# lucaspk512/vrdone

Hardware: AMD Instinct MI355X
Metric: subject-object pairs/sec forward (2048 pairs x 256 frames x 512-d) (higher is better)
Workload: dtype f16x3: f32 products as 3 scaled-f16 MFMA products (~22-bit), f32 accumulate; reference-grade: distance to a float64 run of the reference <= 1.4 x the reference's own float32 error (tests/golden/mask_vrd_f64.npz)

## Files before the change

include/vrdone_hip.h:

```cpp
#ifndef VRDONE_HIP_H
#define VRDONE_HIP_H

#include <stdint.h>

#ifdef __cplusplus
extern "C" {
#endif

#define VRD_ABI_VERSION 36

#define VRD_DETERMINISTIC 1
#define VRD_ERR_SCRATCH (-3)
int vrd_scratch_required(int64_t* floats);

enum vrd_act { VRD_ACT_NONE = 0, VRD_ACT_RELU = 1, VRD_ACT_GELU = 2 };

enum vrd_pair_format { VRD_PAIR_NONE = 0, VRD_PAIR_BF16 = 1, VRD_PAIR_F16 = 2 };
#define VRD_F16_ACT_EXP 4

enum vrd_kernel_id {
    VRD_K_GEMM = 0, VRD_K_LAYERNORM = 1, VRD_K_DWCONV_LN = 2, VRD_K_LOCAL_ATTN = 3,
    VRD_K_ATTN_SMALL = 4, VRD_K_ATTN_FLASH = 5, VRD_K_POOL = 6, VRD_K_MASK_HEAD = 7,
    VRD_K_TRANSPOSE = 8, VRD_K_POSTPROC = 9, VRD_K_GEMM_X3 = 10, VRD_K_GEMM_X3_DMA = 11, VRD_K_GEMM_X3_BIG = 12,
    VRD_K_BACKWARD = 13,
// ... 15 lines not shown
                   float* dst, int64_t ld_dst, int out_pair , int T_src, const int32_t* src_batch,
                   void* stream);
typedef struct {
    const float* const* src;
    const int32_t* lens;
    int32_t P, C_in, T, V, Cc, S, E;
    float* vis;
    float* clip;
    float* so_box;
    float* ent;
    int32_t pair_wide;
} vrd_pack_args;
int vrd_pack_pairs(const vrd_pack_args* a, void* stream);

typedef struct {
    const float* vis;
    const float* clip;
    const float* boxes;
    const int64_t* s_row;
    const int64_t* o_row;
    const int32_t* lens;
    int32_t P, T, V, Cc, stride;
    float w, h;
    float* out_vis;
    float* out_clip;
    float* out_so_box;
    float* out_ent;
    int32_t pair_wide;
    const float* seq_wh;
} vrd_gather_args;
int vrd_gather_pairs(const vrd_gather_args* a, void* stream);

typedef struct {
    const float* vis;
    const float* clip;
    const float* boxes;
    const int64_t* s_row;
    const int64_t* o_row;
    const int32_t* lens;
    const int32_t* lead;
    const float* seq_wh;
    const int32_t* seg_lo;
    const int32_t* seg_hi;
    int32_t P, G, T, V, Cc, stride;
    float* out_vis;
    float* out_clip;
    float* out_so_box;
    float* out_ent;
    uint8_t* out_mask;
    float* out_targets;
    int32_t pair_wide;
} vrd_gather_train_args;
int vrd_gather_train(const vrd_gather_train_args* a, void* stream);

typedef struct {
    const float* streams;
    const float* snippets;
    const int64_t* stream_row;
    const int32_t* lens;
    int32_t P, T, D, L, piece, reach;
    float* out;
} vrd_assemble_args;
int vrd_assemble_pairs(const vrd_assemble_args* a, void* stream);

int vrd_btc_to_bct(const float* src, int64_t ld_src, int B, int C, int T, float* dst, void* stream);

typedef struct {
    const float* A;  int64_t lda;
    const float* W;
    const float* bias;
    float* C;  int64_t ldc;
    int64_t M;  int32_t N;  int32_t Cin;  int32_t taps;  int32_t T;
    int32_t act;
    const uint8_t* row_mask;
    const float* scale;
    const float* res;  int64_t ldres;  int32_t res_masked;
    const float* res2;  int64_t ldres2;
    const uint16_t* W_split;
    int32_t a_pair_width;
    int32_t c_pair;
    const int32_t* row_blocks;
    const int32_t* row_blocks_active;
    int32_t row_block_seg_len;
    int32_t split_fmt;
    const float* w_scale;
    const float* a_scale;
    int32_t products;
} vrd_gemm_args;
int vrd_gemm(const vrd_gemm_args* a, void* stream);
int vrd_gemm_family(const vrd_gemm_args* a);
int vrd_gemm_batch(const vrd_gemm_args* a, int count, void* stream);

int vrd_row_blocks(const uint8_t* mask, int64_t rows, int seg_len, int32_t* order, int32_t* n_active, void* stream);

typedef struct {
    const float* x;
    int64_t ldx;
    int64_t rows;
    int Cin, taps, T, N;
    const float* w;
    const float* bias;
    const uint8_t* row_mask;
    const float* gamma;
    const float* beta;
    int relu;
    float* y;
    int64_t ldy;
    int out_pair;
} vrd_conv_ln_args;
int vrd_conv_ln(const vrd_conv_ln_args* a, void* stream);

int vrd_layernorm(const float* x, int64_t ldx, float* y, int64_t ldy, int64_t rows, int C,
                  const float* gamma, const float* beta, int relu,
                  const float* post_add, int64_t ld_add, int add_period, int out_pair , void* stream);

#define VRD_MAX_SEGS 32
typedef struct {
    int32_t count;
    int32_t n[VRD_MAX_SEGS];
    int32_t T[VRD_MAX_SEGS];
    int64_t row[VRD_MAX_SEGS];
} vrd_row_segs;

typedef struct {
    const float* x;  int64_t ldx;
    const float* x_up;  int64_t ldx_up;
    int32_t B, Tin, C, ksize, stride, group_in;
    const uint8_t* mask_out;
    int32_t n_out;
    const float* w[3];
    const float* bias[3];
    const float* gamma[3];
    const float* beta[3];
    int32_t relu[3];
    float* y[3];
    int64_t ldy[3];
    int32_t out_pair[3];
    const float* pre_gamma;
    const float* pre_beta;
    const float* packed[3];
    const vrd_row_segs* segs;
} vrd_dwconv_ln_args;
int vrd_dwconv_ln(const vrd_dwconv_ln_args* a, void* stream);

int vrd_local_attn(const float* q, const float* k, const float* v, int64_t ld,
                   const uint8_t* mask, const float* rel_pe, int B, int T, int C, int n_head, int half_win,
                   float* out, int64_t ldo, int out_pair, void* stream);
int vrd_local_attn_segs(const float* q, const float* k, const float* v, int64_t ld,
                        const uint8_t* mask, const float* rel_pe, const vrd_row_segs* segs, int C, int n_head, int half_win,
                        float* out, int64_t ldo, int out_pair, void* stream);

int vrd_attention(const float* q, int64_t ldq, const float* k, const float* v, int64_t ldkv,
                  const uint8_t* kv_mask, int B, int Tq, int Tk, int n_head, int head_dim,
                  float* out, int64_t ldo, int algo, int out_pair, void* stream);

int vrd_attention_pair(const float* q, int64_t ldq, const float* k, const float* v, int64_t ldkv,
                       const uint8_t* kv_mask, const uint8_t* q_mask, int B, int Tq, int Tk, int n_head, int head_dim,
                       float* out, int64_t ldo, int out_pair, int pair_fmt, void* stream, int products);

int vrd_maxpool_mask(const float* x, int64_t ldx, int B, int Tin, int C, const uint8_t* mask_in,
                     float* y, int64_t ldy, uint8_t* mask_out, void* stream);

int vrd_mask_head(const float* emb, int64_t ld_emb, const float* feat, int64_t ld_feat,
                  const uint8_t* out_mask, int B, int Q, int T, int Dp, float fill,
                  float* seg, void* stream);

int vrd_postprocess(const float* logits, const float* masks, const int32_t* valid_len,
                    int P, int Q, int K1, int T, int topk,
                    float* top_score, int32_t* top_cat, int32_t* seg_first, int32_t* seg_last,
                    void* stream);

typedef struct {
    const float* cand;
    const float* s_score;
    const float* o_score;
    const int32_t* so_offset;
    const int32_t* so_start;
    const int32_t* so_end;
    const int32_t* video_pairs;
    int32_t n_videos, max_video_pairs, Q, k, feat_stride, pred_min_frames, n_max_pair;
    int32_t* out_count;
    int32_t* out_index;
    float* out_score;
} vrd_select_args;
int vrd_select_triplets(const vrd_select_args* a, void* stream);


int vrd_gemm_wgrad(const float* G, int64_t ldg, const float* X, int64_t ldx, const uint8_t* row_mask, int64_t M, int N, int Cin,
                   int taps, int T, float* dW, float* scratch, int64_t scratch_floats, void* stream, int flags);

int vrd_gemm_wgrad_x3(const float* G, int64_t ldg, const float* X, int64_t ldx, const uint8_t* row_mask, int64_t M, int N, int Cin,
                      int taps, int T, float* dW, float* dbias, float* scratch, int64_t scratch_floats, const float* g_scale,
                      void* stream, int flags);

#define VRD_ABSMAX_SCALE_FLOATS 516
int vrd_absmax_scale(const float* x, int64_t ldx, int64_t rows, int cols, float* scale, void* stream);

int vrd_colsum(const float* a, int64_t lda, const float* b, int64_t ldb, int b_cstride, int b_coffset, int b_rstride, int shift,
               int T, const uint8_t* row_mask, const float* row_scale, int64_t rows, int C, float* out, float* scratch,
               int64_t scratch_floats, void* stream, int flags);

int vrd_dwconv_wgrad(const float* dD, int64_t lddd, const float* x, int64_t ldx, int ksize, int stride, int group_in, int T,
                     const uint8_t* row_mask, int64_t rows, int C, float* dw, float* dbias, float* scratch, int64_t scratch_floats,
                     void* stream, int flags);

int vrd_rowcol_scale(const float* v, int64_t ldv, int64_t rows, int C, const float* col_scale, const float* row_scale,
                     const uint8_t* row_mask, const float* res, int64_t ldres, int res_masked, const float* res2, int64_t ldres2,
                     float* out, int64_t ldo, void* stream);

int vrd_activation(const float* x, int64_t ldx, const float* dy, int64_t lddy, int64_t rows, int C, int act, float* out, int64_t ldo,
            void* stream);

int vrd_layernorm_bwd(const float* x, int64_t ldx, const float* dy, int64_t lddy, int64_t rows, int C, const float* gamma,
                      const float* beta, int relu, float* dx, int64_t lddx, float* dgamma, float* dbeta, float* scratch,
                      int64_t scratch_floats, void* stream, int flags);

typedef struct {
    const float* dD[3];  int64_t lddd[3];
    const float* w[3];
    int32_t n_out, B, Tin, C, ksize, stride, group_in;
    const uint8_t* mask_out;
    float* dx;  int64_t lddx;
    float* dx_up;  int64_t lddx_up;
} vrd_dwconv_bwd_args;
// ... 89 lines not shown
```

vrdone_amd/_hip.py:

```python
import ctypes as C
import os

_HERE = os.path.dirname(os.path.abspath(__file__))
LIB_PATH = os.environ.get("VRDONE_HIP_LIB") or os.path.join(_HERE, "csrc", "libvrdone_hip.so")

ACT_NONE, ACT_RELU, ACT_GELU = 0, 1, 2
PAIR_NONE, PAIR_BF16, PAIR_F16 = 0, 1, 2
F16_ACT_EXP = 4
ABSMAX_SCALE_FLOATS = 516
ADAMW_GROUP_FLOATS = 8
(K_GEMM, K_LAYERNORM, K_DWCONV_LN, K_LOCAL_ATTN, K_ATTN_SMALL, K_ATTN_FLASH, K_POOL, K_MASK_HEAD,
 K_TRANSPOSE, K_POSTPROC, K_GEMM_X3, K_GEMM_X3_DMA, K_GEMM_X3_BIG, K_BACKWARD, K_COUNT) = range(15)
KERNEL_NAMES = ["gemm_f32_mfma", "layernorm", "dwconv_ln", "local_attn", "attn_small", "attn_flash",
                "maxpool_mask", "mask_head", "transpose", "postprocess", "gemm_x3_mfma", "gemm_x3_dma",
                "gemm_x3_big", "backward"]
assert len(KERNEL_NAMES) == K_COUNT

c_f32p = C.c_void_p
c_u8p = C.c_void_p
c_i32p = C.c_void_p


class CriterionArgs(C.Structure):
    _fields_ = [("logits", C.c_void_p * 4), ("masks", C.c_void_p * 4),
                ("n_layers", C.c_int32), ("B", C.c_int32), ("Q", C.c_int32), ("K1", C.c_int32), ("T", C.c_int32), ("G", C.c_int32),
                ("out_valid", C.c_void_p), ("tgt_ids", C.c_void_p), ("tgt_masks", C.c_void_p), ("owner", C.c_void_p),
                ("segs", C.c_void_p), ("scale_range", C.c_float), ("alpha", C.c_float), ("gamma", C.c_float),
                ("w_class", C.c_float), ("w_mask", C.c_float), ("w_dice", C.c_float)]


class CriterionGrads(C.Structure):
    _fields_ = [("logits", C.c_void_p * 4), ("masks", C.c_void_p * 4)]


class GemmArgs(C.Structure):
    _fields_ = [("A", c_f32p), ("lda", C.c_int64), ("W", c_f32p), ("bias", c_f32p),
                ("C", c_f32p), ("ldc", C.c_int64),
                ("M", C.c_int64), ("N", C.c_int32), ("Cin", C.c_int32), ("taps", C.c_int32), ("T", C.c_int32),
                ("act", C.c_int32), ("row_mask", c_u8p), ("scale", c_f32p),
                ("res", c_f32p), ("ldres", C.c_int64), ("res_masked", C.c_int32),
                ("res2", c_f32p), ("ldres2", C.c_int64), ("W_split", C.c_void_p),
                ("a_pair_width", C.c_int32), ("c_pair", C.c_int32),
                ("row_blocks", C.c_void_p), ("row_blocks_active", C.c_void_p), ("row_block_seg_len", C.c_int32),
                ("split_fmt", C.c_int32), ("w_scale", c_f32p), ("a_scale", c_f32p), ("products", C.c_int32)]


MAX_SEGS = 32


class RowSegs(C.Structure):
    _fields_ = [("count", C.c_int32), ("n", C.c_int32 * MAX_SEGS), ("T", C.c_int32 * MAX_SEGS), ("row", C.c_int64 * MAX_SEGS)]

    _made = {}

    @classmethod
    def of(cls, segs):
        key = tuple(segs)
        s = cls._made.get(key)
        if s is None:
            assert 1 <= len(segs) <= MAX_SEGS
            if len(cls._made) > 4096:
                cls._made.clear()
            s = cls._made[key] = cls()
            s.count = len(segs)
            for i, (row, n, T) in enumerate(segs):
                s.row[i], s.n[i], s.T[i] = row, n, T
        return s


class DwconvLnArgs(C.Structure):
    _fields_ = [("x", c_f32p), ("ldx", C.c_int64), ("x_up", c_f32p), ("ldx_up", C.c_int64),
                ("B", C.c_int32), ("Tin", C.c_int32), ("C", C.c_int32), ("ksize", C.c_int32),
                ("stride", C.c_int32), ("group_in", C.c_int32),
                ("mask_out", c_u8p), ("n_out", C.c_int32),
                ("w", c_f32p * 3), ("bias", c_f32p * 3), ("gamma", c_f32p * 3), ("beta", c_f32p * 3),
                ("relu", C.c_int32 * 3), ("y", c_f32p * 3), ("ldy", C.c_int64 * 3), ("out_pair", C.c_int32 * 3),
                ("pre_gamma", c_f32p), ("pre_beta", c_f32p), ("packed", c_f32p * 3), ("segs", C.POINTER(RowSegs))]


class ConvLnArgs(C.Structure):
    _fields_ = [("x", c_f32p), ("ldx", C.c_int64), ("rows", C.c_int64),
                ("Cin", C.c_int32), ("taps", C.c_int32), ("T", C.c_int32), ("N", C.c_int32),
                ("w", c_f32p), ("bias", c_f32p), ("row_mask", c_u8p), ("gamma", c_f32p), ("beta", c_f32p),
                ("relu", C.c_int32), ("y", c_f32p), ("ldy", C.c_int64), ("out_pair", C.c_int32)]


class PackArgs(C.Structure):
    _fields_ = [("src", C.c_void_p), ("lens", C.c_void_p),
                ("P", C.c_int32), ("C_in", C.c_int32), ("T", C.c_int32), ("V", C.c_int32), ("Cc", C.c_int32),
                ("S", C.c_int32), ("E", C.c_int32),
                ("vis", c_f32p), ("clip", c_f32p), ("so_box", c_f32p), ("ent", c_f32p), ("pair_wide", C.c_int32)]


class DwconvBwdArgs(C.Structure):
    _fields_ = [("dD", c_f32p * 3), ("lddd", C.c_int64 * 3), ("w", c_f32p * 3),
                ("n_out", C.c_int32), ("B", C.c_int32), ("Tin", C.c_int32), ("C", C.c_int32), ("ksize", C.c_int32),
                ("stride", C.c_int32), ("group_in", C.c_int32),
                ("mask_out", c_u8p), ("dx", c_f32p), ("lddx", C.c_int64), ("dx_up", c_f32p), ("lddx_up", C.c_int64)]


class BmmArgs(C.Structure):
    _fields_ = [("A", c_f32p), ("a_z0", C.c_int64), ("a_z1", C.c_int64), ("a_row", C.c_int64), ("a_col", C.c_int64),
                ("B", c_f32p), ("b_z0", C.c_int64), ("b_z1", C.c_int64), ("b_row", C.c_int64), ("b_col", C.c_int64),
                ("C", c_f32p), ("c_z0", C.c_int64), ("c_z1", C.c_int64), ("c_row", C.c_int64), ("c_col", C.c_int64),
                ("Z0", C.c_int32), ("Z1", C.c_int32), ("M", C.c_int32), ("N", C.c_int32), ("K", C.c_int32),
                ("alpha", C.c_float), ("accumulate", C.c_int32)]


class SplitJob(C.Structure):
    _fields_ = [("src", c_f32p), ("out", C.c_void_p), ("R", C.c_int32), ("Q", C.c_int32), ("taps", C.c_int32), ("fmt", C.c_int32),
                ("sr", C.c_int64), ("st", C.c_int64), ("sq", C.c_int64), ("scale", c_f32p)]


class GatherArgs(C.Structure):
    _fields_ = [("vis", c_f32p), ("clip", c_f32p), ("boxes", c_f32p), ("s_row", C.c_void_p), ("o_row", C.c_void_p),
                ("lens", C.c_void_p), ("P", C.c_int32), ("T", C.c_int32), ("V", C.c_int32), ("Cc", C.c_int32),
                ("stride", C.c_int32), ("w", C.c_float), ("h", C.c_float),
                ("out_vis", c_f32p), ("out_clip", c_f32p), ("out_so_box", c_f32p), ("out_ent", c_f32p),
                ("pair_wide", C.c_int32), ("seq_wh", c_f32p)]


class GatherTrainArgs(C.Structure):
    _fields_ = [("vis", c_f32p), ("clip", c_f32p), ("boxes", c_f32p), ("s_row", C.c_void_p), ("o_row", C.c_void_p),
                ("lens", C.c_void_p), ("lead", C.c_void_p), ("seq_wh", c_f32p), ("seg_lo", C.c_void_p), ("seg_hi", C.c_void_p),
                ("P", C.c_int32), ("G", C.c_int32), ("T", C.c_int32), ("V", C.c_int32), ("Cc", C.c_int32), ("stride", C.c_int32),
                ("out_vis", c_f32p), ("out_clip", c_f32p), ("out_so_box", c_f32p), ("out_ent", c_f32p), ("out_mask", c_u8p),
                ("out_targets", c_f32p), ("pair_wide", C.c_int32)]


class SelectArgs(C.Structure):
    _fields_ = [("cand", c_f32p), ("s_score", c_f32p), ("o_score", c_f32p), ("so_offset", c_i32p), ("so_start", c_i32p),
                ("so_end", c_i32p), ("video_pairs", c_i32p),
                ("n_videos", C.c_int32), ("max_video_pairs", C.c_int32), ("Q", C.c_int32), ("k", C.c_int32),
                ("feat_stride", C.c_int32), ("pred_min_frames", C.c_int32), ("n_max_pair", C.c_int32),
                ("out_count", c_i32p), ("out_index", c_i32p), ("out_score", c_f32p)]


class AssembleArgs(C.Structure):
    _fields_ = [("streams", c_f32p), ("snippets", c_f32p), ("stream_row", C.c_void_p), ("lens", C.c_void_p),
                ("P", C.c_int32), ("T", C.c_int32), ("D", C.c_int32), ("L", C.c_int32), ("piece", C.c_int32), ("reach", C.c_int32),
                ("out", c_f32p)]


_SIGNATURES = {
    "vrd_abi_version": (C.c_int, []),
    "vrd_last_error": (C.c_char_p, []),
    "vrd_f16_range_flag": (C.c_int, [C.POINTER(C.c_void_p)]),
    "vrd_prof_enable": (C.c_int, [C.c_int]),
    "vrd_prof_reset": (C.c_int, []),
    "vrd_prof_read": (C.c_int, [C.c_int, C.POINTER(C.c_double), C.POINTER(C.c_int64), C.POINTER(C.c_double),
                                C.POINTER(C.c_double)]),
    "vrd_prof_read_skipped": (C.c_int, [C.c_int, C.POINTER(C.c_double)]),
    "vrd_prof_select": (C.c_int, [C.c_uint64]),
    "vrd_bct_to_btc": (C.c_int, [c_f32p, C.c_int, C.c_int, C.c_int, C.c_int, C.c_int, c_f32p, C.c_int64, C.c_int, C.c_int, c_i32p,
                                 C.c_void_p]),
    "vrd_btc_to_bct": (C.c_int, [c_f32p, C.c_int64, C.c_int, C.c_int, C.c_int, c_f32p, C.c_void_p]),
    "vrd_pack_pairs": (C.c_int, [C.POINTER(PackArgs), C.c_void_p]),
    "vrd_gather_pairs": (C.c_int, [C.POINTER(GatherArgs), C.c_void_p]),
    "vrd_gather_train": (C.c_int, [C.POINTER(GatherTrainArgs), C.c_void_p]),
    "vrd_assemble_pairs": (C.c_int, [C.POINTER(AssembleArgs), C.c_void_p]),
# ... 146 lines not shown
```

vrdone_amd/csrc/vrd_gemm.hip:

```cpp
#include "vrd_common.h"
#include "vrd_gemm_epilogue.h"

namespace {

using vrd::f32x16;

constexpr int BM = 128, BN = 128;
constexpr int LDM = 132;

constexpr size_t lds_bytes(int bk) { return (size_t)4 * bk * LDM * sizeof(float); }

template <bool VEC, int TAPS>
__device__ __forceinline__ void load_a(const vrd_gemm_args& p, int64_t r, int t_in_seq, int k, int K, float (&v)[4]) {
    v[0] = v[1] = v[2] = v[3] = 0.f;
    if (r >= p.M) return;
    if (VEC) {
        if (k >= K) return;
        int tap = 0, ci = k;
        if (TAPS == 3) {
            tap = (k >= p.Cin) + (k >= 2 * p.Cin);
            ci = k - tap * p.Cin;
            int tt = t_in_seq + tap - 1;
            if (tt < 0 || tt >= p.T) return;
        }
// ... 154 lines not shown
    constexpr size_t lds = lds_bytes(BK);
    if (lds > 48 * 1024)
        if (int rc = vrd::reserve_lds(reinterpret_cast<const void*>(kern), lds, "vrd_gemm")) return rc;
    hipLaunchKernelGGL(kern, dim3(tiles_m * tiles_n), dim3(256), lds, s, a, tiles_m, tiles_n, a.c_pair == VRD_PAIR_F16 ? vrd::range_flag() : nullptr);
    return 0;
}

template <int BK, bool STAGED>
int launch_bk(const vrd_gemm_args& a, bool vec, int tiles_m, int tiles_n, hipStream_t s) {
    if (a.taps == 1) return vec ? launch_variant<true, 1, BK, STAGED>(a, tiles_m, tiles_n, s)
                                : launch_variant<false, 1, BK, STAGED>(a, tiles_m, tiles_n, s);
    return vec ? launch_variant<true, 3, BK, STAGED>(a, tiles_m, tiles_n, s)
               : launch_variant<false, 3, BK, STAGED>(a, tiles_m, tiles_n, s);
}

}

namespace vrd {
double take_f32_skipped_flops() {
    unsigned long long v = 0, zero = 0;
    if (hipMemcpyFromSymbol(&v, HIP_SYMBOL(g_f32_skipped_kn), sizeof(v)) != hipSuccess) return 0.0;
    (void)hipMemcpyToSymbol(HIP_SYMBOL(g_f32_skipped_kn), &zero, sizeof(zero));
    return 2.0 * BM * (double)v;
}
int launch_gemm_x3(const vrd_gemm_args& a, bool staged, hipStream_t s);
bool gemm_x3_dma_ok(const vrd_gemm_args& a, bool staged);
int launch_gemm_x3_dma(const vrd_gemm_args& a, hipStream_t s);
int launch_gemm_x3_big(const vrd_gemm_args& a, hipStream_t s);
int launch_gemm_x3_big_batch(const vrd_gemm_args* a, int count, hipStream_t s);
}

namespace {
struct X3Choice {
    bool x3, dma, big;
};
X3Choice choose_x3(const vrd_gemm_args* a, bool vec, bool staged) {
    const int K = a->Cin * a->taps;
    const bool x3 = a->a_pair_width > 0 || (a->W_split && vec && (K % 32 == 0) && aligned16(a->W_split));
    static const int dma_env = [] { const char* e = getenv("VRD_X3_DMA"); return e ? atoi(e) : 1; }();
    static const int64_t dma_min_tiles = [] { const char* e = getenv("VRD_X3_DMA_MIN_TILES"); return e ? atoll(e) : 512; }();
    const bool dma = x3 && dma_env && vrd::gemm_x3_dma_ok(*a, staged) &&
                     ((a->M + 127) / 128) * ((a->N + 255) / 256) >= dma_min_tiles;
    static const int64_t big_min_tiles = [] { const char* e = getenv("VRD_X3_BIG_MIN_TILES"); return e ? atoll(e) : 512; }();
    const bool big = dma && a->N >= 256 && K >= 96 && vrd::gemm_epilogue_lean_ok(*a) &&
                     (a->taps == 1 || a->T >= 32) &&
                     (a->products != 1 || (a->Cin % 64 == 0 && K >= 192)) &&
                     (reinterpret_cast<uintptr_t>(a->A) & 127u) == 0 && (reinterpret_cast<uintptr_t>(a->W_split) & 127u) == 0 &&
                     ((a->M + 255) / 256) * ((a->N + 255) / 256) >= big_min_tiles;
    return X3Choice{x3, dma, big};
}
}

namespace {
int validate_gemm_args(const vrd_gemm_args* a) {
    VRD_CHECK_ARG(a->A && a->W && a->C, "vrd_gemm: null operand");
    VRD_CHECK_ARG(a->M >= 0 && a->N > 0 && a->Cin > 0, "vrd_gemm: bad sizes M=%lld N=%d Cin=%d",
                  (long long)a->M, a->N, a->Cin);
    VRD_CHECK_ARG(a->taps == 1 || a->taps == 3, "vrd_gemm: taps must be 1 or 3 (got %d)", a->taps);
    VRD_CHECK_ARG(a->taps == 1 || (a->T > 0 && a->M % a->T == 0),
                  "vrd_gemm: k=3 conv needs M (%lld) to be a multiple of T (%d)", (long long)a->M, a->T);
    VRD_CHECK_ARG(a->lda >= a->Cin && a->ldc >= a->N, "vrd_gemm: leading dimension too small");
    VRD_CHECK_ARG(a->act >= 0 && a->act <= 2, "vrd_gemm: bad activation %d", a->act);
    VRD_CHECK_ARG(!a->res || a->ldres >= a->N, "vrd_gemm: ldres too small");
    VRD_CHECK_ARG(!a->res2 || a->ldres2 >= a->N, "vrd_gemm: ldres2 too small");
    VRD_CHECK_ARG(!a->c_pair || (a->N % 32 == 0 && a->ldc % 32 == 0 && aligned16(a->C)),
                  "vrd_gemm: pair output needs N %% 32 == 0 and rows that start on a 128-byte block");
    VRD_CHECK_ARG(a->a_pair_width == 0 || (a->W_split && a->Cin % 32 == 0 && a->lda % 32 == 0 &&
                                           aligned16(a->A) && aligned16(a->W_split)),
                  "vrd_gemm: pair-row A needs W_split, Cin %% 32 == 0 and rows that start on a 128-byte block");
    VRD_CHECK_ARG(a->split_fmt == 0 || a->split_fmt == VRD_PAIR_BF16 || a->split_fmt == VRD_PAIR_F16, "vrd_gemm: bad split_fmt %d", a->split_fmt);
    VRD_CHECK_ARG(a->split_fmt != VRD_PAIR_F16 || !a->W_split || a->w_scale, "vrd_gemm: a VRD_PAIR_F16 W_split needs w_scale");
    VRD_CHECK_ARG(a->c_pair == VRD_PAIR_NONE || a->c_pair == VRD_PAIR_BF16 || a->c_pair == VRD_PAIR_F16, "vrd_gemm: bad c_pair %d", a->c_pair);
    VRD_CHECK_ARG(!a->a_scale || (a->split_fmt == VRD_PAIR_F16 && a->a_pair_width == 0),
                  "vrd_gemm: a_scale goes with f32-row A in the VRD_PAIR_F16 format");
    VRD_CHECK_ARG(!a->c_pair || !a->W_split || a->c_pair == (a->split_fmt ? a->split_fmt : (int)VRD_PAIR_BF16),
                  "vrd_gemm: pair output (format %d) of a split-precision GEMM must be in its operand format (%d)", a->c_pair, a->split_fmt);
    VRD_CHECK_ARG(a->products == 0 || a->products == 1 || a->products == 3, "vrd_gemm: products must be 0, 1 or 3 (got %d)", a->products);
    VRD_CHECK_ARG(a->products != 1 || (a->split_fmt == VRD_PAIR_F16 && a->W_split),
                  "vrd_gemm: the one-product form (products = 1) needs a VRD_PAIR_F16 W_split (split_fmt %d)", a->split_fmt);
    VRD_CHECK_ARG(!a->row_blocks || (a->row_blocks_active && a->M % 32 == 0 && a->row_block_seg_len >= 8 &&
                                     a->row_block_seg_len % 8 == 0),
                  "vrd_gemm: a row-block list needs its active counts, M %% 32 == 0 and a segment length that is a multiple of 8 (M = %lld, seg_len %d)",
                  (long long)a->M, a->row_block_seg_len);
    return 0;
}
}

static bool gemm_vec(const vrd_gemm_args* a) { return (a->Cin % 4 == 0) && (a->lda % 4 == 0) && aligned16(a->A) && aligned16(a->W); }
static bool gemm_staged(const vrd_gemm_args* a) {
    return (a->ldc % 4 == 0) && aligned16(a->C) && (!a->res || (a->ldres % 4 == 0 && aligned16(a->res))) &&
           (!a->res2 || (a->ldres2 % 4 == 0 && aligned16(a->res2)));
}

extern "C" int vrd_gemm_family(const vrd_gemm_args* a) {
    VRD_CHECK_ARG(a != nullptr, "vrd_gemm_family: null args");
    if (validate_gemm_args(a)) return -1;
    const X3Choice pick = choose_x3(a, gemm_vec(a), gemm_staged(a));
    return pick.big ? VRD_K_GEMM_X3_BIG : pick.dma ? VRD_K_GEMM_X3_DMA : (pick.x3 ? VRD_K_GEMM_X3 : VRD_K_GEMM);
}

extern "C" int vrd_gemm(const vrd_gemm_args* a, void* stream) {
    VRD_CHECK_ARG(a != nullptr, "vrd_gemm: null args");
    if (int rc = validate_gemm_args(a)) return rc;
    if (a->M == 0) return 0;
    const int64_t tiles_m64 = (a->M + BM - 1) / BM;
    const int tiles_n = (a->N + BN - 1) / BN;
    VRD_CHECK_ARG(tiles_m64 * tiles_n < (int64_t)1 << 31, "vrd_gemm: grid too large");
    const int tiles_m = (int)tiles_m64;
    const int K = a->Cin * a->taps;
    const bool vec = gemm_vec(a), staged = gemm_staged(a);
    static const int bk_env = [] { const char* e = getenv("VRD_GEMM_BK"); return e ? atoi(e) : 0; }();
    const int bk = bk_env == 32 ? 32 : 16;
    hipStream_t s = static_cast<hipStream_t>(stream);
    const double flops = 2.0 * (double)a->M * a->N * K;
    const double bytes = 4.0 * ((double)a->M * a->Cin + (double)a->N * K + (double)a->M * a->N *
                                (1.0 + (a->res ? 1.0 : 0.0) + (a->res2 ? 1.0 : 0.0)));
    const X3Choice pick = choose_x3(a, vec, staged);
    const bool x3 = pick.x3, dma = pick.dma, big = pick.big;
    vrd::ProfScope prof(big ? VRD_K_GEMM_X3_BIG : dma ? VRD_K_GEMM_X3_DMA : (x3 ? VRD_K_GEMM_X3 : VRD_K_GEMM), s, flops, bytes);
    if (x3) {
        int rc3 = big ? vrd::launch_gemm_x3_big(*a, s)
                      : dma ? vrd::launch_gemm_x3_dma(*a, s) : vrd::launch_gemm_x3(*a, staged, s);
        if (rc3) return rc3;
        VRD_LAUNCH_CHECK();
        return 0;
    }
    vrd_gemm_args f = *a;
    f.split_fmt = 0;
    f.products = 0;
    f.w_scale = nullptr;
    f.a_scale = nullptr;
    VRD_CHECK_ARG(!f.c_pair || f.c_pair == VRD_PAIR_BF16 || f.c_pair == VRD_PAIR_F16, "vrd_gemm: bad c_pair");
    int rc;
    if (bk == 32) rc = staged ? launch_bk<32, true>(f, vec, tiles_m, tiles_n, s) : launch_bk<32, false>(f, vec, tiles_m, tiles_n, s);
    else          rc = staged ? launch_bk<16, true>(f, vec, tiles_m, tiles_n, s) : launch_bk<16, false>(f, vec, tiles_m, tiles_n, s);
    if (rc) return rc;
    VRD_LAUNCH_CHECK();
    return 0;
}

extern "C" int vrd_gemm_batch(const vrd_gemm_args* a, int count, void* stream) {
    VRD_CHECK_ARG(a != nullptr && count >= 1 && count <= 4, "vrd_gemm_batch: 1..4 problems (got %d)", count);
    for (int i = 0; i < count; ++i)
        if (int rc = validate_gemm_args(&a[i])) return rc;
    for (int i = 1; i < count; ++i)
        VRD_CHECK_ARG((a[i].products == 1) == (a[0].products == 1), "vrd_gemm_batch: every problem needs the same products (%d vs %d)",
                      a[i].products, a[0].products);
    bool same = count > 1 && a[0].M > 0;
    for (int i = 1; i < count && same; ++i) {
        const vrd_gemm_args &x = a[i], &y = a[0];
        same = x.lda == y.lda && x.ldc == y.ldc && x.M == y.M && x.N == y.N && x.Cin == y.Cin && x.taps == y.taps && x.T == y.T &&
               x.act == y.act && x.row_mask == y.row_mask && x.scale == y.scale && x.res == y.res && x.ldres == y.ldres &&
               x.res_masked == y.res_masked && x.res2 == y.res2 && x.ldres2 == y.ldres2 && x.a_pair_width == y.a_pair_width &&
               x.c_pair == y.c_pair && x.row_blocks == y.row_blocks && x.row_blocks_active == y.row_blocks_active &&
               x.row_block_seg_len == y.row_block_seg_len && (x.bias != nullptr) == (y.bias != nullptr) &&
               (x.W_split != nullptr) == (y.W_split != nullptr) && x.split_fmt == y.split_fmt;
    }
    static const int batch_env = [] { const char* e = getenv("VRD_GEMM_BATCH"); return e ? atoi(e) : 1; }();
    if (same && batch_env) {
        bool all_big = true;
        for (int i = 0; i < count && all_big; ++i) {
            const vrd_gemm_args* p = &a[i];
            if (!(p->A && p->W && p->C && p->lda >= p->Cin && p->ldc >= p->N)) { all_big = false; break; }
            const bool vec = (p->Cin % 4 == 0) && (p->lda % 4 == 0) && aligned16(p->A) && aligned16(p->W);
            const bool staged = (p->ldc % 4 == 0) && aligned16(p->C) && (!p->res || (p->ldres % 4 == 0 && aligned16(p->res))) &&
                                (!p->res2 || (p->ldres2 % 4 == 0 && aligned16(p->res2)));
            all_big = choose_x3(p, vec, staged).big && (!p->c_pair || (p->N % 32 == 0 && p->ldc % 32 == 0)) &&
                      (!p->row_blocks || (p->row_blocks_active && p->row_block_seg_len >= 8 && p->row_block_seg_len % 8 == 0));
        }
        if (all_big) {
            hipStream_t s = static_cast<hipStream_t>(stream);
            const int K = a[0].Cin * a[0].taps;
            const double flops = 2.0 * (double)a[0].M * a[0].N * K * count;
            const double bytes = 4.0 * count * ((double)a[0].M * a[0].Cin + (double)a[0].N * K + (double)a[0].M * a[0].N *
                                                (1.0 + (a[0].res ? 1.0 : 0.0) + (a[0].res2 ? 1.0 : 0.0)));
            vrd::ProfScope prof(VRD_K_GEMM_X3_BIG, s, flops, bytes);
            int rc = vrd::launch_gemm_x3_big_batch(a, count, s);
            if (rc) return rc;
            VRD_LAUNCH_CHECK();
            return 0;
        }
    }
    for (int i = 0; i < count; ++i) {
        int rc = vrd_gemm(&a[i], stream);
        if (rc) return rc;
    }
    return 0;
}
```

vrdone_amd/csrc/vrd_gemm_epilogue.h:

```cpp
#pragma once
#include "vrd_common.h"
#include <type_traits>

namespace vrd {

using f32x16 = __attribute__((ext_vector_type(16))) float;
constexpr int STG_PITCH = 64;

typedef float f32x4_t __attribute__((ext_vector_type(4)));
struct acc32q {
    f32x4_t b[2][2];
};
__device__ __forceinline__ void acc_clear(f32x16& a) {
#pragma unroll
    for (int e = 0; e < 16; ++e) a[e] = 0.f;
}
__device__ __forceinline__ void acc_clear(acc32q& a) {
#pragma unroll
    for (int i = 0; i < 2; ++i)
#pragma unroll
        for (int j = 0; j < 2; ++j)
#pragma unroll
            for (int e = 0; e < 4; ++e) a.b[i][j][e] = 0.f;
}
template <typename Fn>
__device__ __forceinline__ void forall32(const f32x16& a, int lane, Fn&& f) {
    const int li = lane & 31, lh = lane >> 5;
#pragma unroll
    for (int e = 0; e < 16; ++e) f((e & 3) + 8 * (e >> 2) + 4 * lh, li, a[e]);
}
template <typename Fn>
__device__ __forceinline__ void forall32(const acc32q& a, int lane, Fn&& f) {
    const int lc = lane & 15, lq = lane >> 4;
#pragma unroll
    for (int bi = 0; bi < 2; ++bi)
#pragma unroll
        for (int bj = 0; bj < 2; ++bj)
#pragma unroll
            for (int j = 0; j < 4; ++j) f(16 * bi + 4 * lq + j, 16 * bj + lc, a.b[bi][bj][j]);
}

__device__ __forceinline__ float epilogue_value(const vrd_gemm_args& p, float v, float mk, float scale, float r1, float rmk,
                                                float r2) {
    if (p.act == VRD_ACT_RELU) v = fmaxf(v, 0.f);
    else if (p.act == VRD_ACT_GELU) v = gelu_erf(v);
    return v * mk * scale + r1 * rmk + r2;
}

struct EpiCols {
    float bias[4], scale[4];
    float alpha;
};
__device__ __forceinline__ float acc_alpha(const vrd_gemm_args& p) {
    if (!(p.split_fmt == VRD_PAIR_F16 && p.w_scale)) return 1.0f;
    const float alpha = uniform_load(p.w_scale);
    return (p.a_scale && p.a_pair_width == 0) ? alpha * F16_ACT_SCALE * uniform_load(p.a_scale + 1) : alpha;
}
__device__ __forceinline__ EpiCols load_epi_cols(const vrd_gemm_args& p, int nw, int lane) {
    EpiCols c;
    c.alpha = acc_alpha(p);
    const int n = nw + (lane & 15) * 4;
#pragma unroll
    for (int j = 0; j < 4; ++j) c.bias[j] = 0.f, c.scale[j] = 1.f;
    if (n + 3 < p.N) {
        if (p.bias) {
            const float4 b = gload4(p.bias + n);
            c.bias[0] = b.x, c.bias[1] = b.y, c.bias[2] = b.z, c.bias[3] = b.w;
        }
        if (p.scale) {
            const float4 b = gload4(p.scale + n);
            c.scale[0] = b.x, c.scale[1] = b.y, c.scale[2] = b.z, c.scale[3] = b.w;
        }
    }
    return c;
}

__device__ __forceinline__ EpiCols load_epi_cols_async(const vrd_gemm_args& p, int nw, int lane) {
    EpiCols c;
    c.alpha = acc_alpha(p);
    const int n = nw + (lane & 15) * 4;
    float4 b = make_float4(0.f, 0.f, 0.f, 0.f), sc = make_float4(1.f, 1.f, 1.f, 1.f);
    if (n + 3 < p.N) {
        if (p.bias) asm volatile("global_load_dwordx4 %0, %1, off" : "=v"(b) : "v"(p.bias + n) : "memory");
        if (p.scale) asm volatile("global_load_dwordx4 %0, %1, off" : "=v"(sc) : "v"(p.scale + n) : "memory");
    }
    c.bias[0] = b.x, c.bias[1] = b.y, c.bias[2] = b.z, c.bias[3] = b.w;
    c.scale[0] = sc.x, c.scale[1] = sc.y, c.scale[2] = sc.z, c.scale[3] = sc.w;
    return c;
}

template <bool ROWIN, int ACT, int SLAB, int ROWS, typename Transposer>
__device__ __forceinline__ void gemm_epilogue_lean_tr(const vrd_gemm_args& p, Transposer&& transpose_into, float* stg, int64_t mw,
                                                      int64_t mw1, int nw, int lane, const EpiCols& cols, unsigned* rflag = nullptr) {
    RangeTrack rt;
    const int64_t hop = mw1 - (mw + 32);
    const int c4 = (lane & 15) * 4, rb0 = lane >> 4;
    const int n = nw + c4;
    const int64_t m_lane = mw + rb0;
    const bool pair = p.c_pair != 0;
    char* const c_lane = reinterpret_cast<char*>(p.C + m_lane * p.ldc) + (pair ? pair_index(n) * 2 : n * 4);
    const float* const r1_lane = (ROWIN && p.res) ? p.res + m_lane * p.ldres + n : nullptr;
    const float* const r2_lane = (ROWIN && p.res2) ? p.res2 + m_lane * p.ldres2 + n : nullptr;
    const unsigned char* const mk_lane = (ROWIN && p.row_mask) ? p.row_mask + m_lane : nullptr;
    const int64_t c_step = p.ldc * 16, r1_step = p.ldres * 4, r2_step = p.ldres2 * 4;
    const int64_t c_hop = hop * p.ldc * 4;
    struct RowIn {
        unsigned char mb[4];
        float4 r1[4], r2[4];
    };
    auto fetch = [&](int pass) {
        RowIn in;
        if (ROWIN) {
            if (p.row_mask) {
#pragma unroll
                for (int j = 0; j < 4; ++j) in.mb[j] = *as_global(mk_lane + pass * 16 + 4 * j + (pass >= 2 ? hop : 0));
            }
            if (p.res) {
#pragma unroll
                for (int j = 0; j < 4; ++j)
                    in.r1[j] = gload4(r1_lane + (pass * 4 + j) * r1_step + (pass >= 2 ? hop * p.ldres : 0));
            }
            if (p.res2) {
#pragma unroll
                for (int j = 0; j < 4; ++j)
                    in.r2[j] = gload4(r2_lane + (pass * 4 + j) * r2_step + (pass >= 2 ? hop * p.ldres2 : 0));
            }
        }
        return in;
    };
    constexpr int NPASS = ROWS / 16;
    RowIn q0 = fetch(0), q1 = fetch(1);
    unsigned rd_addr[4];
    {
        typedef __attribute__((address_space(3))) const float* lds_cf;
#pragma unroll
        for (int j = 0; j < 4; ++j) rd_addr[j] = (unsigned)reinterpret_cast<uintptr_t>((lds_cf)(stg + (rb0 + 4 * j) * STG_PITCH + (c4 ^ (16 * j))));
    }
    transpose_into(stg, SLAB == 64 ? -1 : 0);
#pragma unroll
    for (int pass = 0; pass < NPASS; ++pass) {
        if (SLAB == 32 && pass == 2) transpose_into(stg, 1);
        const RowIn cur = q0;
        q0 = q1;
        if (pass + 2 < NPASS) q1 = fetch(pass + 2);
        float v[4][4];
        float4 tr[4];
        {
            constexpr int PASS_OFF = (SLAB == 64 ? 1 : 0);
            const int poff = (PASS_OFF ? pass : (pass & 1)) * 16 * STG_PITCH * 4;
            asm volatile("ds_read_b128 %0, %4 offset:%8\n\tds_read_b128 %1, %5 offset:%8\n\tds_read_b128 %2, %6 offset:%8\n\tds_read_b128 %3, %7 offset:%8\n\t"
                         "s_waitcnt lgkmcnt(0)"
                         : "=&v"(tr[0]), "=&v"(tr[1]), "=&v"(tr[2]), "=&v"(tr[3])
                         : "v"(rd_addr[0]), "v"(rd_addr[1]), "v"(rd_addr[2]), "v"(rd_addr[3]), "n"(poff)
                         : "memory");
        }
#pragma unroll
        for (int j = 0; j < 4; ++j) {
            const float4 t = tr[j];
            v[j][0] = fmaf(t.x, cols.alpha, cols.bias[0]), v[j][1] = fmaf(t.y, cols.alpha, cols.bias[1]);
            v[j][2] = fmaf(t.z, cols.alpha, cols.bias[2]), v[j][3] = fmaf(t.w, cols.alpha, cols.bias[3]);
        }
        if (ACT == VRD_ACT_GELU) {
#pragma unroll
            for (int j = 0; j < 4; ++j)
#pragma unroll
                for (int c = 0; c < 4; c += 2) {
                    f32x2_t t2;
                    t2.x = v[j][c], t2.y = v[j][c + 1];
                    t2 = gelu_erf2(t2);
                    v[j][c] = t2.x, v[j][c + 1] = t2.y;
                }
        }
        if (ROWIN) {
            float mk[4] = {1.f, 1.f, 1.f, 1.f};
            if (p.row_mask) {
#pragma unroll
                for (int j = 0; j < 4; ++j) mk[j] = (float)cur.mb[j];
            }
            if (p.row_mask || p.scale) {
#pragma unroll
                for (int j = 0; j < 4; ++j)
#pragma unroll
                    for (int c = 0; c < 4; ++c) v[j][c] *= mk[j] * cols.scale[c];
            }
            if (p.res) {
#pragma unroll
                for (int j = 0; j < 4; ++j) {
                    const float rmk = p.res_masked ? mk[j] : 1.f;
                    v[j][0] += cur.r1[j].x * rmk, v[j][1] += cur.r1[j].y * rmk;
                    v[j][2] += cur.r1[j].z * rmk, v[j][3] += cur.r1[j].w * rmk;
                }
            }
            if (p.res2) {
#pragma unroll
                for (int j = 0; j < 4; ++j) {
                    v[j][0] += cur.r2[j].x, v[j][1] += cur.r2[j].y;
                    v[j][2] += cur.r2[j].z, v[j][3] += cur.r2[j].w;
                }
            }
        }
        if (pair) {
            if (p.c_pair == VRD_PAIR_F16) {
#pragma unroll
                for (int j = 0; j < 4; ++j) {
                    char* const rowp = c_lane + (pass * 4 + j) * c_step + (pass >= 2 ? c_hop : 0);
                    f16x4_t h, l;
                    split_n<true>(v[j], h, l, &rt);
                    *as_global(reinterpret_cast<f16x4_t*>(rowp)) = h;
                    *as_global(reinterpret_cast<f16x4_t*>(rowp + 64)) = l;
                }
            } else {
#pragma unroll
                for (int j = 0; j < 4; ++j) {
                    char* const rowp = c_lane + (pass * 4 + j) * c_step + (pass >= 2 ? c_hop : 0);
                    bf16x4_t h, l;
                    split_n<false>(v[j], h, l);
                    *as_global(reinterpret_cast<bf16x4_t*>(rowp)) = h;
                    *as_global(reinterpret_cast<bf16x4_t*>(rowp + 64)) = l;
                }
            }
        } else {
#pragma unroll
            for (int j = 0; j < 4; ++j)
                gstore4(c_lane + (pass * 4 + j) * c_step + (pass >= 2 ? c_hop : 0), make_float4(v[j][0], v[j][1], v[j][2], v[j][3]));
        }
    }
    if (p.c_pair == VRD_PAIR_F16) rt.report(rflag, RANGE_GEMM_OUT);
}

template <bool ROWIN, int ACT, int SLAB = 64>
__device__ __forceinline__ void gemm_epilogue_lean16(const vrd_gemm_args& p, const f32x4_t (&acc)[4][4], float* stg, int64_t mw,
                                                     int64_t mw1, int nw, int lane, const EpiCols& cols, unsigned* rflag = nullptr) {
    const int lc = lane & 15, lq = lane >> 4;
    gemm_epilogue_lean_tr<ROWIN, ACT, SLAB, 64>(
        p,
        [&](float* slab, int half) {
#pragma unroll
            for (int ti = 0; ti < 4; ++ti) {
                if (half >= 0 && (ti >> 1) != half) continue;
                const int r0 = half < 0 ? ti * 16 : (ti & 1) * 16;
#pragma unroll
                for (int tj = 0; tj < 4; ++tj)
#pragma unroll
                    for (int j = 0; j < 4; ++j) slab[(r0 + 4 * lq + j) * STG_PITCH + (tj ^ lq) * 16 + lc] = acc[ti][tj][j];
            }
        },
        stg, mw, mw1, nw, lane, cols, rflag);
}

inline bool gemm_epilogue_lean_ok(const vrd_gemm_args& a) {
    auto al16 = [](const void* q) { return (reinterpret_cast<uintptr_t>(q) & 15u) == 0; };
    return a.M % 64 == 0 && a.N % 64 == 0 && (a.act == VRD_ACT_NONE || a.act == VRD_ACT_GELU) &&
           !(a.act == VRD_ACT_GELU && (a.row_mask || a.scale || a.res || a.res2)) && al16(a.bias) && al16(a.scale);
}

template <bool STAGED, int SLAB_ROWS = 32, typename Acc>
__device__ __forceinline__ void gemm_epilogue(const vrd_gemm_args& p, const Acc (&acc)[2][2], float* smem, int64_t mw,
                                              int nw, int wave, int lane, unsigned* rflag = nullptr, int64_t mw1 = -1) {
    if (mw1 < 0) mw1 = mw + 32;
    auto rowbase = [&](int mi) { return mi ? mw1 : mw; };
    RangeTrack rt;
    constexpr bool SWZ = std::is_same<Acc, acc32q>::value;
    if (STAGED) {
        float* stg = smem + wave * (SLAB_ROWS * STG_PITCH);
        const int c4 = (lane & 15) * 4, rb0 = lane >> 4;
        const int n = nw + c4;
        const bool nfull = n + 3 < p.N;
        const float alpha = acc_alpha(p);
        float bias[4] = {0.f, 0.f, 0.f, 0.f}, scale[4] = {1.f, 1.f, 1.f, 1.f};
        if (nfull && ((reinterpret_cast<uintptr_t>(p.bias) | reinterpret_cast<uintptr_t>(p.scale)) & 15) == 0) {
            if (p.bias) {
                const float4 b = *reinterpret_cast<const float4*>(p.bias + n);
                bias[0] = b.x, bias[1] = b.y, bias[2] = b.z, bias[3] = b.w;
            }
            if (p.scale) {
                const float4 b = *reinterpret_cast<const float4*>(p.scale + n);
                scale[0] = b.x, scale[1] = b.y, scale[2] = b.z, scale[3] = b.w;
            }
        } else {
#pragma unroll
            for (int j = 0; j < 4; ++j)
                if (n + j < p.N) {
                    if (p.bias) bias[j] = p.bias[n + j];
                    if (p.scale) scale[j] = p.scale[n + j];
                }
        }
        const bool row_inputs = p.row_mask || p.res || p.res2;
        const bool ragged = __any(n < p.N && !nfull);
        struct RowIn {
            float mk[4];
            float4 r1[4], r2[4];
        };
        auto fetch = [&](int pass) {
            RowIn in;
#pragma unroll
            for (int j = 0; j < 4; ++j) {
                in.mk[j] = 1.f;
                in.r1[j] = make_float4(0.f, 0.f, 0.f, 0.f);
                in.r2[j] = in.r1[j];
            }
            if (!row_inputs) return in;
            const int64_t mr = rowbase(pass >> 1) + rb0 + (pass & 1) * 16;
            if (!ragged) {
                const int nc = n < p.N ? n : 0;
                unsigned char mb[4];
                int64_t mc[4];
#pragma unroll
                for (int j = 0; j < 4; ++j) mc[j] = (mr + 4 * j < p.M) ? mr + 4 * j : p.M - 1;
                if (p.row_mask) {
#pragma unroll
                    for (int j = 0; j < 4; ++j) mb[j] = p.row_mask[mc[j]];
                }
                if (p.res) {
#pragma unroll
                    for (int j = 0; j < 4; ++j) in.r1[j] = *reinterpret_cast<const float4*>(p.res + mc[j] * p.ldres + nc);
                }
                if (p.res2) {
#pragma unroll
                    for (int j = 0; j < 4; ++j) in.r2[j] = *reinterpret_cast<const float4*>(p.res2 + mc[j] * p.ldres2 + nc);
                }
                if (p.row_mask) {
#pragma unroll
                    for (int j = 0; j < 4; ++j) in.mk[j] = (float)mb[j];
                }
                return in;
            }
#pragma unroll
            for (int j = 0; j < 4; ++j) {
                const int64_t m = mr + 4 * j;
                const bool ok = m < p.M && n < p.N;
// ... 126 lines not shown
```

vrdone_amd/csrc/vrd_gemm_x3_big.hip:

```cpp
#include "vrd_common.h"
#include "vrd_gemm_epilogue.h"
#include <cstdlib>
#include <type_traits>

namespace {

typedef __attribute__((address_space(3))) void* lds_ptr_t;

constexpr int TM = 256, TN = 256;
constexpr int ROWB = 128;
constexpr int A_STAGE = TM * ROWB, W_STAGE = TN * ROWB;
constexpr int NA_STG = 3, NW_STG = 2;
__attribute__((unused)) constexpr int W_RING = NA_STG * A_STAGE;
constexpr size_t BIG_LDS = (size_t)NA_STG * A_STAGE + (size_t)NW_STG * W_STAGE;
__attribute__((unused)) constexpr int PER = 4;
__device__ unsigned long long g_big_skipped_kn;

#ifndef VRD_LAB_STAMP
#define LAB_STAMP(slot)
#define LAB_REAL(slot)
#define LAB_PHASE_DECL
#define LAB_PHASE(i)
#define LAB_PHASE_FLUSH(grp)
#else
// ... 15 lines not shown
    } while (0)
#endif

__device__ constexpr int swz(int row) { return (row >> 1) & 7; }

struct BigBatch {
    const float* A[3];
    const uint16_t* W_split[3];
    const float* bias[3];
    float* C[3];
    const float* w_scale[3];
};

struct BigKArgs {
    vrd_gemm_args p;
    int tiles_m, tiles_n;
    BigBatch bb;
    int stagger;
    int count;
    unsigned* rflag;
};
typedef const __attribute__((address_space(4))) unsigned* kargs_ptr_t;
template <typename T>
__device__ __forceinline__ T load_karg(kargs_ptr_t base, int byte_off) {
    constexpr int N = (sizeof(T) + 3) / 4;
    unsigned tmp[N];
#pragma unroll
    for (int i = 0; i < N; ++i) tmp[i] = base[byte_off / 4 + i];
    T out;
    __builtin_memcpy(&out, tmp, sizeof(T));
    return out;
}

template <int TAPS, bool PERSIST, bool F16, int WH, int NPROD>
__device__ __forceinline__ void gemm_x3_big_body() {
    static_assert(NPROD == 3 || (NPROD == 1 && F16), "the one-product form exists for the f16 format only");
#if defined(__HIP_DEVICE_COMPILE__)
    constexpr bool LO = NPROD == 3;
    constexpr int KB = LO ? 1 : 2;
    constexpr int NQ = LO ? 12 : 8;
    typedef typename vrd::SplitFmt<F16>::x8 e16x8;
    kargs_ptr_t kp = (kargs_ptr_t)__builtin_amdgcn_kernarg_segment_ptr();
    vrd_gemm_args p;
    int tiles_m, tiles_n, K, nkt, nwg, nblk;
    const int32_t* rb;
    int64_t a_pstride, w_pstride;
    int zsel = PERSIST ? 0 : (int)blockIdx.y;
    auto reload = [&]() __attribute__((always_inline)) {
        if (PERSIST) asm volatile("" : "+s"(kp));
        p = load_karg<vrd_gemm_args>(kp, offsetof(BigKArgs, p));
        tiles_m = load_karg<int>(kp, offsetof(BigKArgs, tiles_m));
        tiles_n = load_karg<int>(kp, offsetof(BigKArgs, tiles_n));
        if (zsel) {
            const BigBatch bb = load_karg<BigBatch>(kp, offsetof(BigKArgs, bb));
            const int z = zsel;
            p.A = z == 1 ? bb.A[0] : z == 2 ? bb.A[1] : bb.A[2];
            p.w_scale = z == 1 ? bb.w_scale[0] : z == 2 ? bb.w_scale[1] : bb.w_scale[2];
            p.W_split = z == 1 ? bb.W_split[0] : z == 2 ? bb.W_split[1] : bb.W_split[2];
            p.bias = z == 1 ? bb.bias[0] : z == 2 ? bb.bias[1] : bb.bias[2];
            p.C = z == 1 ? bb.C[0] : z == 2 ? bb.C[1] : bb.C[2];
        }
        K = p.Cin * TAPS;
        nkt = K / (32 * KB);
        nwg = tiles_m * tiles_n;
        nblk = (int)(p.M >> 5);
        rb = p.row_blocks;
        a_pstride = p.lda * 32, w_pstride = (int64_t)K * 32;
    };
    reload();
    const int stagger = PERSIST ? 0 : load_karg<int>(kp, offsetof(BigKArgs, stagger));
    unsigned* rflag = nullptr;
    if (stagger && blockIdx.y == 0 && blockIdx.x < 256) {
        const int n = ((blockIdx.x >> 3) & 31) * stagger;
        for (int i = 0; i < n; ++i) __builtin_amdgcn_s_sleep(16);
    }
    extern __shared__ __attribute__((aligned(16))) float smem[];
    char* const lds = reinterpret_cast<char*>(smem);
    const int tid = threadIdx.x;
    const int lane = tid & 63;
    const int wave = WH * 4 + (__builtin_amdgcn_readfirstlane(tid >> 6) & 3);
    const int wm = WH, wn = wave & 3;
    auto blk_of = [&](int slot) { return slot < nblk ? (rb ? vrd::uniform_load(rb + slot) : slot) : -1; };
    struct Tile {
        int tm, n0;
        bool contract;
    };
    auto tile_of = [&](int vb_) {
        const int xcd = vb_ & 7, q = nwg >> 3, rem = nwg & 7;
        const int lid = (xcd < rem ? xcd * (q + 1) : rem * (q + 1) + (xcd - rem) * q) + (vb_ >> 3);
        Tile t;
        t.tm = lid / tiles_n;
        t.n0 = (lid - t.tm * tiles_n) * TN;
        t.contract = true;
        if (rb) {
            const int seg_len = p.row_block_seg_len;
            const int seg = (t.tm * 8) / seg_len;
            t.contract = t.tm * 8 < nblk && t.tm * 8 - seg * seg_len < vrd::uniform_load(p.row_blocks_active + seg);
        }
        return t;
    };
    const int rin = lane >> 3, pch = lane & 7;
    const int row0 = wave * PER * 8 + rin;
    const int chunk0 = (pch ^ swz(row0)) * 16;
    unsigned va[2], vw[2];
    auto lane_offsets = [&]() {
        const unsigned a_lane = (unsigned)rin * (unsigned)(p.lda * 4), w_lane = (unsigned)rin * (unsigned)(K * 4);
        if (LO) {
            va[0] = a_lane + chunk0, va[1] = a_lane + (chunk0 ^ 64);
            vw[0] = w_lane + chunk0, vw[1] = w_lane + (chunk0 ^ 64);
        } else {
            const unsigned c0 = chunk0 >> 4, c1 = c0 ^ 4;
            const unsigned s0 = (c0 & 3) * 16 + (c0 >> 2) * 128, s1 = (c1 & 3) * 16 + (c1 >> 2) * 128;
            va[0] = a_lane + s0, va[1] = a_lane + s1;
            vw[0] = w_lane + s0, vw[1] = w_lane + s1;
        }
    };
    lane_offsets();
    struct Src {
        int tseq0, a_in, w_last;
        __amdgpu_buffer_rsrc_t ra, rw;
    };
    auto src_of = [&](const Tile& t) {
        const int my_blk = blk_of(t.tm * 8 + wave);
        const int64_t a_row = (int64_t)(my_blk < 0 ? 0 : my_blk) * 32 + rin;
        Src r;
        r.tseq0 = (TAPS == 3) ? (int)(a_row % p.T) : 0;
        r.a_in = my_blk < 0 ? 0 : PER;
        const int w_in = (p.N - t.n0 - wave * PER * 8 + 7) / 8;
        r.w_last = (w_in > 0 ? (w_in < PER ? w_in : PER) : 1) - 1;
        const int64_t a_row_u = (int64_t)(my_blk < 0 ? 0 : my_blk) * 32 - (TAPS == 3 ? 1 : 0);
        r.ra = __builtin_amdgcn_make_buffer_rsrc(const_cast<float*>(p.A + a_row_u * p.lda), 0, 0x80000000u, 0x00020000);
        r.rw = __builtin_amdgcn_make_buffer_rsrc(
            const_cast<char*>(reinterpret_cast<const char*>(p.W_split) + (int64_t)(t.n0 + (w_in > 0 ? wave * PER * 8 : 0)) * K * 4), 0,
            0x80000000u, 0x00020000);
        return r;
    };
    auto issue_w1 = [&](const Src& c, int gk, int ks, int i) {
        char* const dst = lds + W_RING + (gk % NW_STG) * W_STAGE + wave * PER * 1024;
        __builtin_amdgcn_raw_ptr_buffer_load_lds(c.rw, (lds_ptr_t)(dst + i * 1024), 16, vw[i & 1],
                                                 (i < c.w_last ? i : c.w_last) * (int)w_pstride + ks * 128 * KB, 0, 0);
    };
    auto issue_a1 = [&](const Src& c, int gk, int ks, int i) {
        char* const dst = lds + (gk % NA_STG) * A_STAGE + wave * PER * 1024;
        const int k0 = ks * 32 * KB;
        int tap = 0, ci0 = k0;
        unsigned vo = va[i & 1];
        if (TAPS == 3) {
            tap = (k0 >= p.Cin) + (k0 >= 2 * p.Cin);
            ci0 = k0 - tap * p.Cin;
            int tt = c.tseq0 + 8 * i;
            if (tt >= p.T) tt -= p.T;
            tt += tap - 1;
            if (tt < 0 || tt >= p.T || i >= c.a_in) vo = 0x80000000u;
        }
        __builtin_amdgcn_raw_ptr_buffer_load_lds(c.ra, (lds_ptr_t)(dst + i * 1024), 16, vo,
                                                 i * (int)a_pstride + tap * (int)(p.lda * 4) + ci0 * 4, 0, 0);
    };
    auto issue_w = [&](const Src& c, int gk, int ks) {
#pragma unroll
        for (int i = 0; i < PER; ++i) issue_w1(c, gk, ks, i);
    };
    auto issue_a = [&](const Src& c, int gk, int ks) {
#pragma unroll
        for (int i = 0; i < PER; ++i) issue_a1(c, gk, ks, i);
    };

    bool staged = false;
    bool stored_all = false;
    int g0 = 0;
    const int count = PERSIST ? load_karg<int>(kp, offsetof(BigKArgs, count)) : 1;
    int vq = blockIdx.x, vb = blockIdx.x;
#ifdef VRD_BIG_NOCARRY
    constexpr bool CARRY = false;
#else
    constexpr bool CARRY = true;
#endif
    Tile nt_keep = Tile{0, 0, false};
    Src nx_keep = src_of(nt_keep);
    do {
    if (PERSIST) {
        zsel = (vq >= nwg) + (vq >= 2 * nwg) + (vq >= 3 * nwg);
        vb = vq - zsel * nwg;
        if (vq != (int)blockIdx.x || zsel) reload();
    }
    LAB_STAMP(0);
    LAB_REAL(4);
    const Tile tile = (PERSIST && staged && CARRY) ? nt_keep : tile_of(vb);
    const int tm = tile.tm, n0 = tile.n0;
    const bool contract = tile.contract;
    const Src cur = (PERSIST && staged && CARRY) ? nx_keep : src_of(tile);
    bool next_staged = false;
    Src nx = cur;
    if (PERSIST && contract && vb + (int)gridDim.x < nwg) {
        const Tile nt = tile_of(vb + (int)gridDim.x);
        if (nt.contract) {
            nx = src_of(nt);
            next_staged = true;
            nt_keep = nt;
        }
    }
    nx_keep = nx;
    if (!contract && tid == 0 && tm * 8 < nblk)
        atomicAdd(&g_big_skipped_kn, (unsigned long long)K * (unsigned)(p.N - n0 < TN ? p.N - n0 : TN));

    const int l15 = lane & 15, l4 = lane >> 4;
    int a_hi_off = (wm * 128 + l15) * ROWB + ((l4 ^ swz(l15)) * 16), a_lo_off = a_hi_off ^ 64;
    int w_hi_off = W_RING + (wn * 64 + l15) * ROWB + ((l4 ^ swz(l15)) * 16), w_lo_off = w_hi_off ^ 64;
    asm volatile("" : "+v"(a_hi_off), "+v"(a_lo_off), "+v"(w_hi_off), "+v"(w_lo_off));

    const vrd::EpiCols cols = vrd::load_epi_cols_async(p, n0 + wn * 64, lane);
    vrd::f32x4_t acc[8][4];
    if (!contract) {
        float z;
        asm volatile("v_mov_b32 %0, 0" : "=v"(z));
#pragma unroll
        for (int i = 0; i < 8; ++i)
#pragma unroll
            for (int j = 0; j < 4; ++j)
#pragma unroll
                for (int e = 0; e < 4; ++e) acc[i][j][e] = z;
    }

    struct AF { e16x8 hi, lo; };
    struct WF { e16x8 hi[4], lo[4]; };
    auto load_a = [&](const char* sa, int mi) {
        AF f;
        f.hi = *reinterpret_cast<const e16x8*>(sa + a_hi_off + mi * 16 * ROWB);
        f.lo = *reinterpret_cast<const e16x8*>(sa + a_lo_off + mi * 16 * ROWB);
        return f;
    };
    auto load_w1 = [&](const char* sw, int t, WF& f) {
        f.hi[t] = *reinterpret_cast<const e16x8*>(sw + w_hi_off + t * 16 * ROWB);
        f.lo[t] = *reinterpret_cast<const e16x8*>(sw + w_lo_off + t * 16 * ROWB);
    };
    if (contract) {
    if (!(PERSIST && staged)) {
        issue_a(cur, g0, 0);
        issue_w(cur, g0, 0);
        issue_a(cur, g0 + 1, 1);
        issue_w(cur, g0 + 1, 1);
        LAB_STAMP(1);
        asm volatile("s_waitcnt vmcnt(%0)" ::"n"(2 * PER) : "memory");
    } else {
        issue_w(cur, g0 + 1, 1);
        LAB_STAMP(1);
        if (stored_all) asm volatile("s_waitcnt vmcnt(%0)" ::"n"(2 * PER + 32) : "memory");
        else asm volatile("s_waitcnt vmcnt(%0)" ::"n"(2 * PER) : "memory");
    }
    LAB_STAMP(6);
    __builtin_amdgcn_s_barrier();
    LAB_STAMP(7);
    WF w_cur;
#pragma unroll
    for (int t = 0; t < 4; ++t) load_w1(lds + (g0 % NW_STG) * W_STAGE, t, w_cur);
    AF a_cur = load_a(lds + (g0 % NA_STG) * A_STAGE, 0), a_nxt = a_cur;
    LAB_PHASE_DECL;
    enum { POS_FIRST, POS_STEADY, POS_PEN, POS_LAST };
    auto kstep = [&](int kt, auto pos_c) __attribute__((always_inline)) {
        constexpr int POS = decltype(pos_c)::value;
        auto dma_slot = [&](int kt_open, int d, bool w_ok, bool a_ok) {
            if (d < PER) {
                if (w_ok) issue_w1(cur, g0 + kt_open + 2, kt_open + 2, d);
            } else {
                if (a_ok) issue_a1(cur, g0 + kt_open + 3, kt_open + 3, d - PER);
            }
        };
        auto dma_slot_next = [&](int j_w, int j_a, int d) {
            if (d < PER) issue_w1(nx, g0 + nkt + j_w, j_w, d);
            else issue_a1(nx, g0 + nkt + j_a, j_a, d - PER);
        };
        const char* sa = lds + ((g0 + kt) % NA_STG) * A_STAGE;
        const char* sa1 = lds + ((g0 + kt + 1) % NA_STG) * A_STAGE;
        const char* sw1 = lds + ((g0 + kt + 1) % NW_STG) * W_STAGE;
        constexpr bool last = POS == POS_LAST;
#pragma unroll
        for (int g = 0; g < 8; ++g) {
            if (g == 0) __builtin_amdgcn_s_setprio(3);
            if (g == 2) __builtin_amdgcn_s_setprio(2);
            if (g == 4) __builtin_amdgcn_s_setprio(1);
            if (g == 6) __builtin_amdgcn_s_setprio(0);
            if (g < 7) a_nxt = load_a(sa, g + 1);
            if (g == 7 && !last) a_nxt = load_a(sa1, 0);
            auto dma_of_group = [&]() __attribute__((always_inline)) {
                __builtin_amdgcn_sched_barrier(0);
#ifdef VRD_LAB_NODMA
                if (POS == POS_STEADY) return;
#endif
                if (g < 7) {
                    if (POS == POS_FIRST) {
                        if (g < PER) issue_a1(cur, g0 + 2, 2, g);
                    } else if (POS == POS_STEADY) {
                        dma_slot(kt - 1, g + 1, true, true);
                    } else if (POS == POS_PEN) {
                        if (g + 1 < PER) dma_slot(kt - 1, g + 1, true, false);
                        else if (PERSIST) dma_slot_next(0, 0, g + 1);
                    } else if (POS == POS_LAST && PERSIST) {
                        dma_slot_next(0, 1, g + 1);
                    }
                } else if (!last) {
                    if (POS == POS_PEN && PERSIST) dma_slot_next(0, 0, 0);
                    else dma_slot(kt, 0, POS != POS_PEN, false);
                }
                __builtin_amdgcn_sched_barrier(0);
            };
            constexpr bool blockmajor = !last;
#pragma unroll
            for (int q = 0; q < NQ; ++q) {
                const int pr = LO ? ((blockmajor && g == 7) ? q % 3 : q >> 2) : 0;
                const int kb = LO ? 0 : ((blockmajor && g == 7) ? q & 1 : q >> 2);
                const int t = LO ? ((blockmajor && g == 7) ? q / 3 : q & 3) : ((blockmajor && g == 7) ? q >> 1 : q & 3);
                const bool a_lo = LO ? pr == 0 : kb == 1, w_lo = LO ? pr == 1 : kb == 1;
                const bool chain0 = LO ? pr == 0 : kb == 0, w_done = LO ? pr == 2 : kb == 1;
                const vrd::f32x4_t zero4 = {0.f, 0.f, 0.f, 0.f};
                acc[g][t] = vrd::mfma16(a_lo ? a_cur.lo : a_cur.hi, w_lo ? w_cur.lo[t] : w_cur.hi[t],
                                        (POS == POS_FIRST && chain0) ? zero4 : acc[g][t]);
                if (blockmajor && g == 7 && w_done) load_w1(sw1, t, w_cur);
                if ((q == NQ / 2 - 1 && WH == 0) || (q == NQ - 1 && WH == 1)) dma_of_group();
            }
            a_cur = a_nxt;
            if (g == 6 && !last) {
                asm volatile("s_waitcnt lgkmcnt(0)" ::: "memory");
                LAB_PHASE(3);
                if (POS != POS_PEN || PERSIST) asm volatile("s_waitcnt vmcnt(%0)" ::"n"(PER) : "memory");
                else asm volatile("s_waitcnt vmcnt(0)" ::: "memory");
                LAB_PHASE(0);
                __builtin_amdgcn_sched_barrier(0);
                __builtin_amdgcn_s_barrier();
                __builtin_amdgcn_sched_barrier(0);
                LAB_PHASE(1);
            }
        }
    };
    kstep(0, std::integral_constant<int, POS_FIRST>{});
    for (int kt = 1; kt + 2 < nkt; ++kt) kstep(kt, std::integral_constant<int, POS_STEADY>{});
    kstep(nkt - 2, std::integral_constant<int, POS_PEN>{});
    kstep(nkt - 1, std::integral_constant<int, POS_LAST>{});
    LAB_PHASE_FLUSH(WH);
    __builtin_amdgcn_s_setprio(0);
    }
#ifdef VRD_LAB_STAMP
    asm volatile("" ::"v"(acc[0][0][0]));
#endif
    if (!contract) asm volatile("s_waitcnt vmcnt(0)" ::: "memory");
    asm volatile("s_waitcnt lgkmcnt(0)" ::: "memory");
    __builtin_amdgcn_s_barrier();
    LAB_STAMP(2);
    rflag = load_karg<unsigned*>(kp, offsetof(BigKArgs, rflag));
    if (PERSIST) {
        reload();
        staged = next_staged;
    }
    const int slab_a = ((g0 + nkt + 2) % NA_STG) * A_STAGE, slab_w = W_RING + ((g0 + nkt + 1) % NW_STG) * W_STAGE;
    float* const stg = PERSIST ? smem + ((wave < 4 ? slab_a : slab_w - 4 * (32 * vrd::STG_PITCH * 4)) + wave * (32 * vrd::STG_PITCH * 4)) / 4
                               : smem + wave * (64 * vrd::STG_PITCH);
    bool all_stored = true;
    constexpr int SLAB = PERSIST ? 32 : 64;
    int lane_e = lane;
    asm volatile("" : "+v"(lane_e));
#pragma unroll
    for (int hm = 0; hm < 2; ++hm) {
        const int slot = tm * 8 + wm * 4 + hm * 2;
        const int blk_a = blk_of(slot), blk_b = blk_of(slot + 1);
        const int nw = n0 + wn * 64;
        if (blk_a < 0 || nw >= p.N) {
            all_stored = false;
            continue;
        }
        const int64_t mw = (int64_t)blk_a * 32, mw1 = (int64_t)blk_b * 32;
        const bool rowin = !PERSIST && (p.row_mask || p.scale || p.res || p.res2);
        vrd::f32x4_t part[4][4];
#pragma unroll
        for (int i = 0; i < 4; ++i)
#pragma unroll
            for (int j = 0; j < 4; ++j) part[i][j] = acc[4 * hm + i][j];
        if (rowin) vrd::gemm_epilogue_lean16<true, VRD_ACT_NONE, SLAB>(p, part, stg, mw, mw1, nw, lane_e, cols, rflag);
        else if (p.act == VRD_ACT_GELU) vrd::gemm_epilogue_lean16<false, VRD_ACT_GELU, SLAB>(p, part, stg, mw, mw1, nw, lane_e, cols, rflag);
        else vrd::gemm_epilogue_lean16<false, VRD_ACT_NONE, SLAB>(p, part, stg, mw, mw1, nw, lane_e, cols, rflag);
    }
    LAB_STAMP(3);
    LAB_REAL(5);
    if (PERSIST) {
        asm volatile("s_waitcnt lgkmcnt(0)" ::: "memory");
        __builtin_amdgcn_s_barrier();
    }
    stored_all = all_stored;
    g0 = (g0 + nkt) % 6;
    vq += (int)gridDim.x;
    } while (PERSIST && vq < nwg * count);
    if (PERSIST) asm volatile("s_waitcnt vmcnt(0)" ::: "memory");
#endif
}

template <int TAPS, bool PERSIST, bool F16 = false, int NPROD = 3>
__global__ __launch_bounds__(512) void gemm_x3_big_kernel(BigKArgs ka_unused_) {
    if (__builtin_amdgcn_readfirstlane(threadIdx.x >> 8)) gemm_x3_big_body<TAPS, PERSIST, F16, 1, NPROD>();
    else gemm_x3_big_body<TAPS, PERSIST, F16, 0, NPROD>();
}

}

namespace vrd {

template <int TAPS, bool PERSIST, bool F16 = false, int NPROD = 3>
static int launch_big_one(const vrd_gemm_args& a, hipStream_t s, const BigBatch& bb = BigBatch{}, int count = 1) {
    auto kern = gemm_x3_big_kernel<TAPS, PERSIST, F16, NPROD>;
    if (int rc = reserve_lds(reinterpret_cast<const void*>(kern), BIG_LDS, "vrd_gemm(bf16x3 256x256)")) return rc;
    const int tiles_m = (int)((a.M + TM - 1) / TM), tiles_n = (a.N + TN - 1) / TN;
    const int nwg = tiles_m * tiles_n;
    static const int stagger = [] { const char* e = getenv("VRD_BIG_STAGGER"); return e ? atoi(e) : 2; }();
    const int n_cu = PERSIST ? device_cu_count() : 0;
    BigKArgs ka;
    ka.p = a, ka.tiles_m = tiles_m, ka.tiles_n = tiles_n, ka.bb = bb, ka.stagger = (PERSIST || nwg < 512) ? 0 : stagger;
    ka.rflag = a.c_pair == VRD_PAIR_F16 ? range_flag() : nullptr;
    ka.count = count;
    if (PERSIST) hipLaunchKernelGGL(kern, dim3(nwg * count < n_cu ? nwg * count : n_cu), dim3(512), BIG_LDS, s, ka);
    else hipLaunchKernelGGL(kern, dim3(nwg, count), dim3(512), BIG_LDS, s, ka);
    return 0;
}

static bool big_persist(const vrd_gemm_args& a) {
    static const int persist = [] { const char* e = getenv("VRD_BIG_PERSIST"); return e ? atoi(e) : 1; }();
    return persist && a.taps == 1 && a.Cin >= 96 && !(a.row_mask || a.scale || a.res || a.res2);
}

static int launch_big_any(const vrd_gemm_args& a, hipStream_t s, const BigBatch& bb, int count) {
    const bool f16 = a.split_fmt == VRD_PAIR_F16;
    if (f16 && a.products == 1) {
        if (big_persist(a)) return launch_big_one<1, true, true, 1>(a, s, bb, count);
        return a.taps == 1 ? launch_big_one<1, false, true, 1>(a, s, bb, count) : launch_big_one<3, false, true, 1>(a, s, bb, count);
    }
    if (big_persist(a)) return f16 ? launch_big_one<1, true, true>(a, s, bb, count) : launch_big_one<1, true, false>(a, s, bb, count);
    if (f16) return a.taps == 1 ? launch_big_one<1, false, true>(a, s, bb, count) : launch_big_one<3, false, true>(a, s, bb, count);
    return a.taps == 1 ? launch_big_one<1, false, false>(a, s, bb, count) : launch_big_one<3, false, false>(a, s, bb, count);
}

int launch_gemm_x3_big_batch(const vrd_gemm_args* a, int count, hipStream_t s) {
    BigBatch bb{};
    for (int i = 1; i < count; ++i) {
        bb.A[i - 1] = a[i].A;
        bb.W_split[i - 1] = a[i].W_split;
        bb.bias[i - 1] = a[i].bias;
        bb.C[i - 1] = a[i].C;
        bb.w_scale[i - 1] = a[i].w_scale;
    }
    return launch_big_any(a[0], s, bb, count);
}

double take_big_skipped_flops() {
    unsigned long long v = 0, zero = 0;
    if (hipMemcpyFromSymbol(&v, HIP_SYMBOL(g_big_skipped_kn), sizeof(v)) != hipSuccess) return 0.0;
    (void)hipMemcpyToSymbol(HIP_SYMBOL(g_big_skipped_kn), &zero, sizeof(zero));
    return 2.0 * TM * (double)v;
}

int launch_gemm_x3_big(const vrd_gemm_args& a, hipStream_t s) { return launch_big_any(a, s, BigBatch{}, 1); }

}
```

vrdone_amd/csrc/vrd_rowops.hip:

```cpp
#include "vrd_common.h"
#include "vrd_box_feats.h"
#include <cmath>

namespace {

constexpr float LN_EPS = 1e-5f;

__device__ __forceinline__ float4 ld4(const float* p) { return *reinterpret_cast<const float4*>(p); }
__device__ __forceinline__ void st4(float* p, float4 v) { *reinterpret_cast<float4*>(p) = v; }
__device__ __forceinline__ float4 f4add(float4 a, float4 b) { return make_float4(a.x + b.x, a.y + b.y, a.z + b.z, a.w + b.w); }

__global__ __launch_bounds__(256) void bct_to_btc_kernel(const float* __restrict__ src, int C_total, int T, int c0,
                                                         int count, float* __restrict__ dst, int64_t ld_dst, int pair, int T_src,
                                                         const int32_t* __restrict__ src_batch, unsigned* rflag) {
    __shared__ float tile[64][65];
    vrd::RangeTrack rt;
    const int b = blockIdx.z, ct = blockIdx.y * 64, tt = blockIdx.x * 64;
    const int tx = threadIdx.x & 63, ty = threadIdx.x >> 6;
    const float* s = src + ((int64_t)(src_batch ? src_batch[b] : b) * C_total + c0) * T_src;
    for (int c = ty; c < 64; c += 4)
        tile[c][tx] = (ct + c < count && tt + tx < T) ? s[(int64_t)(ct + c) * T_src + tt + tx] : 0.f;
    __syncthreads();
    for (int t = ty; t < 64; t += 4)
        if (tt + t < T && ct + tx < count) {
// ... 229 lines not shown
    const int lane = threadIdx.x & 63;
    constexpr int RG = 4;
    int64_t grp = (int64_t)blockIdx.x * 4 + __builtin_amdgcn_readfirstlane(threadIdx.x >> 6);
    const int64_t stride = (int64_t)gridDim.x * 4;
    const int half = p.taps / 2;
    const int lrow = lane / p.Cin, lci = lane - lrow * p.Cin;
    auto load_in = [&](int64_t g) {
        const int64_t r = g * RG - half + lrow;
        float val = 0.f;
        if (lrow < RG + 2 * half && r >= 0 && r < p.rows) val = p.x[r * p.ldx + lci];
        return val;
    };
    float xin = grp * RG < p.rows ? load_in(grp) : 0.f;
    for (; grp * RG < p.rows; grp += stride) {
        const int64_t row0 = grp * RG;
        const float xcur = xin;
        if ((grp + stride) * RG < p.rows) xin = load_in(grp + stride);
        float4 v[RG][NV];
        int t[RG];
#pragma unroll
        for (int j = 0; j < RG; ++j) {
            t[j] = (int)((row0 + j) % p.T);
#pragma unroll
            for (int i = 0; i < NV; ++i) v[j][i] = *reinterpret_cast<const float4*>(cl_lds + K * N + lane_chan<NV, WIDE>(i, lane));
        }
        for (int tap = 0; tap < p.taps; ++tap) {
            for (int ci = 0; ci < p.Cin; ++ci) {
                const float* wk = cl_lds + (tap * p.Cin + ci) * N;
                float4 w[NV];
#pragma unroll
                for (int i = 0; i < NV; ++i) w[i] = *reinterpret_cast<const float4*>(wk + lane_chan<NV, WIDE>(i, lane));
#pragma unroll
                for (int j = 0; j < RG; ++j) {
                    const int tt = t[j] + tap - half;
                    const bool ok = tt >= 0 && tt < p.T && row0 + j < p.rows;
                    const float xl = __builtin_bit_cast(float, __builtin_amdgcn_readlane(__builtin_bit_cast(int, xcur), (j + tap) * p.Cin + ci));
                    const float xv = ok ? xl : 0.f;
#pragma unroll
                    for (int i = 0; i < NV; ++i) {
                        v[j][i].x = fmaf(w[i].x, xv, v[j][i].x); v[j][i].y = fmaf(w[i].y, xv, v[j][i].y);
                        v[j][i].z = fmaf(w[i].z, xv, v[j][i].z); v[j][i].w = fmaf(w[i].w, xv, v[j][i].w);
                    }
                }
            }
        }
#pragma unroll
        for (int j = 0; j < RG; ++j) {
            const int64_t row = row0 + j;
            if (row >= p.rows) break;
            if (p.row_mask) {
                const float mk = (float)vrd::uniform_load(p.row_mask + row);
#pragma unroll
                for (int i = 0; i < NV; ++i) v[j][i].x *= mk, v[j][i].y *= mk, v[j][i].z *= mk, v[j][i].w *= mk;
            }
            if (p.gamma) {
                ln_rows<NV, WIDE>(v[j], p.gamma, p.beta, lane, p.relu != 0);
            } else if (p.relu) {
#pragma unroll
                for (int i = 0; i < NV; ++i) {
                    v[j][i].x = fmaxf(v[j][i].x, 0.f); v[j][i].y = fmaxf(v[j][i].y, 0.f);
                    v[j][i].z = fmaxf(v[j][i].z, 0.f); v[j][i].w = fmaxf(v[j][i].w, 0.f);
                }
            }
            float* yr = p.y + row * p.ldy;
            if (WIDE && p.out_pair) {
                vrd::store_pair8(yr, lane * 8, v[j][0], v[j][NV - 1], p.out_pair, &rt);
            } else {
#pragma unroll
                for (int i = 0; i < NV; ++i) {
                    const int c = lane_chan<NV, WIDE>(i, lane);
                    if (p.out_pair) vrd::store_pair4(yr, c, N, v[j][i], p.out_pair, &rt);
                    else st4(yr + c, v[j][i]);
                }
            }
        }
    }
    rt.report(rflag, vrd::RANGE_LAYERNORM);
}

constexpr int DW_RW = 16;

template <int NV, int KS, int GIN>
__global__ __launch_bounds__(256) void dwconv_ln_kernel(vrd_dwconv_ln_args p, int Tout_u, int strips_per_seq, int strips_per_wave, int rw, unsigned* rflag,
                                                        vrd::SegTable sg) {
    vrd::RangeTrack rt;
    constexpr int C = 256 * NV, NT = GIN * KS, SETF = (NT + 3) * C;
    constexpr bool WIDE = NV == 2 && GIN == 1;
    extern __shared__ __attribute__((aligned(16))) float dw_lds[];
    const int lane = threadIdx.x & 63, wave = __builtin_amdgcn_readfirstlane(threadIdx.x >> 6);
    for (int o = 0; o < p.n_out; ++o) {
        float* const ls = dw_lds + o * SETF;
        if (p.packed[o]) {
            for (int idx = threadIdx.x * 4; idx < SETF; idx += 1024) st4(ls + idx, ld4(p.packed[o] + idx));
            continue;
        }
        for (int idx = threadIdx.x; idx < C * NT; idx += 256) ls[(idx % NT) * C + idx / NT] = p.w[o][idx];
        for (int c = threadIdx.x; c < C; c += 256) {
            ls[NT * C + c] = p.bias[o] ? p.bias[o][c] : 0.f;
            ls[(NT + 1) * C + c] = p.gamma[o] ? p.gamma[o][c] : 1.f;
            ls[(NT + 2) * C + c] = p.gamma[o] ? p.beta[o][c] : 0.f;
        }
    }
    const float* const pre = dw_lds + p.n_out * SETF;
    if (p.pre_gamma)
        for (int c = threadIdx.x; c < C; c += 256) {
            dw_lds[p.n_out * SETF + c] = p.pre_gamma[c];
            dw_lds[p.n_out * SETF + C + c] = p.pre_beta[c];
        }
    __syncthreads();
    const int nwg = gridDim.x, bid = blockIdx.x;
    const int xcd = bid & 7, qq = nwg >> 3, rem = nwg & 7;
    const int lid = (xcd < rem ? xcd * (qq + 1) : rem * (qq + 1) + (xcd - rem) * qq) + (bid >> 3);
    for (int si = 0; si < strips_per_wave; ++si) {
    const int64_t ws = ((int64_t)lid * 4 + wave) * strips_per_wave + si;
    int Tin, Tout, to0;
    int64_t xrow0, urow0, orow0;
    if (sg.count) {
        int g, b, strip;
        if (!vrd::seg_find(sg, ws, g, b, strip)) break;
        Tin = sg.T[g], Tout = Tin / p.stride, to0 = strip * rw;
        xrow0 = sg.row[g] + (int64_t)b * Tin;
        urow0 = sg.row[g] / 2 + (int64_t)b * (Tin / 2);
        orow0 = sg.row[g] / p.stride + (int64_t)b * Tout;
    } else {
        const int b = (int)(ws / strips_per_seq);
        if (b >= p.B) break;
        Tin = p.Tin, Tout = Tout_u, to0 = (int)(ws - (int64_t)b * strips_per_seq) * rw;
        xrow0 = (int64_t)b * Tin, urow0 = (int64_t)b * (Tin / 2), orow0 = (int64_t)b * Tout;
    }
    const int to1 = min(to0 + rw, Tout);

    struct Row {
        float4 v[NV][GIN];
    };
    auto load_row = [&](int ti) {
        Row r;
        const bool ok = ti >= 0 && ti < Tin;
#pragma unroll
        for (int i = 0; i < NV; ++i)
#pragma unroll
            for (int g = 0; g < GIN; ++g) {
                float4 v = make_float4(0.f, 0.f, 0.f, 0.f);
                if (ok) {
                    const int64_t coff = (int64_t)GIN * lane_chan<NV, WIDE>(i, lane) + 4 * g;
                    v = ld4(p.x + (xrow0 + ti) * p.ldx + coff);
                    if (p.x_up) v = f4add(v, ld4(p.x_up + (urow0 + (ti >> 1)) * p.ldx_up + coff));
                }
                r.v[i][g] = v;
            }
        if (GIN == 1 && p.pre_gamma && ok) {
            float4 t[NV];
#pragma unroll
            for (int i = 0; i < NV; ++i) t[i] = r.v[i][0];
            ln_rows<NV, WIDE>(t, pre, pre + C, lane, false);
#pragma unroll
            for (int i = 0; i < NV; ++i) r.v[i][0] = t[i];
        }
        return r;
    };
    if (p.mask_out) {
        const int64_t r0 = orow0 + to0;
        const bool mine = lane < to1 - to0 && p.mask_out[r0 + lane] != 0;
        if (!__any(mine)) {
#pragma unroll
            for (int o = 0; o < 3; ++o) {
                if (o >= p.n_out) break;
                const float* const lb = dw_lds + o * SETF + (NT + 2) * C;
                float4 val[NV];
#pragma unroll
                for (int i = 0; i < NV; ++i) {
                    val[i] = *reinterpret_cast<const float4*>(lb + lane_chan<NV, WIDE>(i, lane));
                    if (p.relu[o]) {
                        val[i].x = fmaxf(val[i].x, 0.f); val[i].y = fmaxf(val[i].y, 0.f);
                        val[i].z = fmaxf(val[i].z, 0.f); val[i].w = fmaxf(val[i].w, 0.f);
                    }
                }
                for (int to = to0; to < to1; ++to) {
                    const int64_t row = orow0 + to;
                    if (WIDE && p.out_pair[o]) {
                        vrd::store_pair8(p.y[o] + row * p.ldy[o], lane * 8, val[0], val[NV - 1], p.out_pair[o], &rt);
                    } else {
#pragma unroll
                        for (int i = 0; i < NV; ++i) {
                            const int c = lane_chan<NV, WIDE>(i, lane);
                            if (p.out_pair[o]) vrd::store_pair4(p.y[o] + row * p.ldy[o], c, 256 * NV, val[i], p.out_pair[o], &rt);
                            else st4(p.y[o] + row * p.ldy[o] + c, val[i]);
                        }
                    }
                }
            }
            continue;
        }
    }
    Row win[KS];
#pragma unroll
    for (int k = 0; k < KS; ++k) win[k] = load_row(p.stride * to0 + k - KS / 2);
    for (int to = to0; to < to1; ++to) {
        Row nxt[2];
        const int tn = p.stride * (to + 1) - KS / 2;
        const bool more = to + 1 < to1;
        if (KS == 1) {
            if (more) nxt[0] = load_row(tn);
        } else if (p.stride == 1) {
            if (more) nxt[0] = load_row(tn + 2);
        } else {
            if (more) {
                nxt[0] = load_row(tn + 1);
                nxt[1] = load_row(tn + 2);
            }
        }
        const int64_t row = orow0 + to;
        const float mk = p.mask_out ? (float)p.mask_out[row] : 1.f;
#pragma unroll
        for (int o = 0; o < 3; ++o) {
            if (o >= p.n_out) break;
            const float* const ls = dw_lds + o * SETF;
            float4 acc[NV];
#pragma unroll
            for (int i = 0; i < NV; ++i) {
                const int c = lane_chan<NV, WIDE>(i, lane);
                float4 r = *reinterpret_cast<const float4*>(ls + NT * C + c);
#pragma unroll
                for (int k = 0; k < KS; ++k) {
                    if (GIN == 1) {
                        const float4 w = *reinterpret_cast<const float4*>(ls + k * C + c);
                        const float4 v = win[k].v[i][0];
                        r.x += w.x * v.x; r.y += w.y * v.y; r.z += w.z * v.z; r.w += w.w * v.w;
                    } else {
                        const float4 w0 = *reinterpret_cast<const float4*>(ls + (0 * KS + k) * C + c);
                        const float4 w1 = *reinterpret_cast<const float4*>(ls + (1 * KS + k) * C + c);
                        const float4 v0 = win[k].v[i][0], v1 = win[k].v[i][GIN - 1];
                        r.x += w0.x * v0.x + w1.x * v0.y;
                        r.y += w0.y * v0.z + w1.y * v0.w;
                        r.z += w0.z * v1.x + w1.z * v1.y;
                        r.w += w0.w * v1.z + w1.w * v1.w;
                    }
                }
                acc[i] = make_float4(r.x * mk, r.y * mk, r.z * mk, r.w * mk);
            }
            if (p.gamma[o]) {
                ln_rows<NV, WIDE>(acc, ls + (NT + 1) * C, ls + (NT + 2) * C, lane, p.relu[o] != 0);
            } else if (p.relu[o]) {
#pragma unroll
                for (int i = 0; i < NV; ++i) {
                    acc[i].x = fmaxf(acc[i].x, 0.f); acc[i].y = fmaxf(acc[i].y, 0.f);
                    acc[i].z = fmaxf(acc[i].z, 0.f); acc[i].w = fmaxf(acc[i].w, 0.f);
                }
            }
            if (WIDE && p.out_pair[o]) {
// ... 210 lines not shown
    VRD_CHECK_ARG(B > 0 && B <= 65535 && T > 0 && C > 0 && ld_src >= C, "vrd_btc_to_bct: bad shape");
    hipStream_t s = static_cast<hipStream_t>(stream);
    vrd::ProfScope prof(VRD_K_TRANSPOSE, s, 0.0, 8.0 * B * (double)C * T);
    dim3 grid((T + 63) / 64, (C + 63) / 64, B);
    hipLaunchKernelGGL(btc_to_bct_kernel, grid, dim3(256), 0, s, src, ld_src, C, T, dst);
    VRD_LAUNCH_CHECK();
    return 0;
}

int vrd_layernorm(const float* x, int64_t ldx, float* y, int64_t ldy, int64_t rows, int C, const float* gamma,
                  const float* beta, int relu, const float* post_add, int64_t ld_add, int add_period, int out_pair,
                  void* stream) {
    VRD_CHECK_ARG(x && y && gamma && beta, "vrd_layernorm: null pointer");
    VRD_CHECK_ARG(C == 256 || C == 512, "vrd_layernorm: C must be 256 or 512 (got %d)", C);
    VRD_CHECK_ARG(ldx >= C && ldy >= C && ldx % 4 == 0 && ldy % 4 == 0 && aligned16(x) && aligned16(y) &&
                      aligned16(gamma) && aligned16(beta),
                  "vrd_layernorm: rows must be 16-byte aligned");
    VRD_CHECK_ARG(!post_add || (add_period > 0 && ld_add % 4 == 0 && aligned16(post_add)), "vrd_layernorm: bad post_add");
    if (rows <= 0) return 0;
    hipStream_t s = static_cast<hipStream_t>(stream);
    vrd::ProfScope prof(VRD_K_LAYERNORM, s, 0.0, 8.0 * (double)rows * C);
    unsigned* const rflag = out_pair == VRD_PAIR_F16 ? vrd::range_flag() : nullptr;
    static const int64_t max_blocks = [] { const char* e = getenv("VRD_LN_BLOCKS"); return e ? atoll(e) : 8192; }();
    const int64_t want = (rows + 3) / 4;
    dim3 grid((unsigned)(max_blocks > 0 && want > max_blocks ? max_blocks : want));
    if (C == 256)
        hipLaunchKernelGGL(layernorm_kernel<1>, grid, dim3(256), 0, s, x, ldx, y, ldy, rows, gamma, beta, relu, post_add, ld_add, add_period, out_pair, rflag);
    else
        hipLaunchKernelGGL(layernorm_kernel<2>, grid, dim3(256), 0, s, x, ldx, y, ldy, rows, gamma, beta, relu, post_add, ld_add, add_period, out_pair, rflag);
    VRD_LAUNCH_CHECK();
    return 0;
}

int vrd_conv_ln(const vrd_conv_ln_args* a, void* stream) {
    VRD_CHECK_ARG(a && a->x && a->w && a->y, "vrd_conv_ln: null pointer");
    VRD_CHECK_ARG(a->N == 256 || a->N == 512, "vrd_conv_ln: N must be 256 or 512 (got %d)", a->N);
    VRD_CHECK_ARG((a->taps == 1 || a->taps == 3) && a->Cin > 0 && a->Cin * a->taps <= CL_MAXK && (4 + a->taps - 1) * a->Cin <= 64,
                  "vrd_conv_ln: taps in {1, 3}, taps * Cin <= %d and (3 + taps) * Cin <= 64 (got %d x %d)", CL_MAXK, a->taps, a->Cin);
    VRD_CHECK_ARG(a->rows >= 0 && a->T > 0 && a->rows % a->T == 0 && a->ldx >= a->Cin, "vrd_conv_ln: bad rows / T / ldx");
    VRD_CHECK_ARG((a->gamma == nullptr) == (a->beta == nullptr), "vrd_conv_ln: gamma and beta go together");
    VRD_CHECK_ARG(a->ldy >= a->N && a->ldy % 4 == 0 && aligned16(a->y) && aligned16(a->gamma) && aligned16(a->beta),
                  "vrd_conv_ln: output rows and LayerNorm parameters must be 16-byte aligned");
    VRD_CHECK_ARG(!a->out_pair || (a->ldy % 32 == 0 && (a->out_pair == VRD_PAIR_BF16 || a->out_pair == VRD_PAIR_F16)),
                  "vrd_conv_ln: pair output needs rows that start on a 128-byte block");
    if (a->rows == 0) return 0;
    hipStream_t s = static_cast<hipStream_t>(stream);
    const int K = a->Cin * a->taps;
    vrd::ProfScope prof(VRD_K_LAYERNORM, s, 2.0 * (double)a->rows * a->N * K, 4.0 * (double)a->rows * (a->N + a->Cin));
    unsigned* const rflag = a->out_pair == VRD_PAIR_F16 ? vrd::range_flag() : nullptr;
    const size_t lds = (size_t)(K + 1) * a->N * sizeof(float);
    const int64_t want = (a->rows + 15) / 16;
    dim3 grid((unsigned)(want > 4096 ? 4096 : want));
    if (a->N == 256) {
        if (lds > 48 * 1024)
            if (int rc = vrd::reserve_lds(reinterpret_cast<const void*>(conv_ln_kernel<1>), lds, "vrd_conv_ln")) return rc;
        hipLaunchKernelGGL(conv_ln_kernel<1>, grid, dim3(256), lds, s, *a, rflag);
    } else {
        if (lds > 48 * 1024)
            if (int rc = vrd::reserve_lds(reinterpret_cast<const void*>(conv_ln_kernel<2>), lds, "vrd_conv_ln")) return rc;
        hipLaunchKernelGGL(conv_ln_kernel<2>, grid, dim3(256), lds, s, *a, rflag);
    }
    VRD_LAUNCH_CHECK();
    return 0;
}

int vrd_dwconv_ln(const vrd_dwconv_ln_args* a, void* stream) {
    VRD_CHECK_ARG(a && a->x, "vrd_dwconv_ln: null args");
    VRD_CHECK_ARG(a->C == 256 || a->C == 512, "vrd_dwconv_ln: C must be 256 or 512 (got %d)", a->C);
    VRD_CHECK_ARG(a->ksize == 1 || a->ksize == 3, "vrd_dwconv_ln: ksize must be 1 or 3");
    VRD_CHECK_ARG(a->stride == 1 || a->stride == 2, "vrd_dwconv_ln: stride must be 1 or 2");
    VRD_CHECK_ARG(a->group_in == 1 || (a->group_in == 2 && a->C == 256 && a->ksize == 3),
                  "vrd_dwconv_ln: group_in=2 is only built for C=256, ksize=3");
    VRD_CHECK_ARG(a->segs || (a->B > 0 && a->Tin > 0 && a->Tin % a->stride == 0), "vrd_dwconv_ln: Tin %% stride != 0");
    VRD_CHECK_ARG(a->n_out >= 1 && a->n_out <= 3, "vrd_dwconv_ln: n_out must be 1..3");
    VRD_CHECK_ARG((a->pre_gamma == nullptr) == (a->pre_beta == nullptr) && (!a->pre_gamma || (a->group_in == 1 && !a->x_up)),
                  "vrd_dwconv_ln: input LayerNorm needs gamma and beta, group_in == 1 and no x_up");
    VRD_CHECK_ARG(a->ldx >= (int64_t)a->C * a->group_in && a->ldx % 4 == 0 && aligned16(a->x), "vrd_dwconv_ln: bad x layout");
    VRD_CHECK_ARG(!a->x_up || (a->Tin % 2 == 0 && a->ldx_up % 4 == 0 && aligned16(a->x_up)), "vrd_dwconv_ln: bad x_up layout");
    for (int o = 0; o < a->n_out; ++o) {
        VRD_CHECK_ARG((a->w[o] || a->packed[o]) && a->y[o] && aligned16(a->w[o]) && aligned16(a->packed[o]) && aligned16(a->y[o]) &&
                          a->ldy[o] % 4 == 0 && a->ldy[o] >= a->C,
                      "vrd_dwconv_ln: bad output set %d", o);
        VRD_CHECK_ARG((a->gamma[o] == nullptr) == (a->beta[o] == nullptr), "vrd_dwconv_ln: gamma/beta mismatch");
    }
    vrd::SegTable sg;
    sg.count = 0;
    int64_t rows_in = (int64_t)a->B * a->Tin;
    int Tmax = a->Tin;
    if (a->segs) {
        const int even = (a->x_up || a->stride == 2) ? 2 : 1;
        VRD_CHECK_ARG(vrd::seg_table(sg, a->segs, even, 16) >= 0, "vrd_dwconv_ln: bad row groups (1..%d groups, T %% %d == 0)", VRD_MAX_SEGS, even);
        rows_in = 0, Tmax = 0;
        for (int g = 0; g < sg.count; ++g) {
            VRD_CHECK_ARG(sg.row[g] % even == 0, "vrd_dwconv_ln: a group's first row must be even with stride 2 / x_up");
            rows_in += (int64_t)sg.n[g] * sg.T[g];
            Tmax = sg.T[g] > Tmax ? sg.T[g] : Tmax;
        }
    }
    const int Tout = Tmax / a->stride;
    const int64_t rows = rows_in / a->stride;
    hipStream_t s = static_cast<hipStream_t>(stream);
    vrd::ProfScope prof(VRD_K_DWCONV_LN, s, 0.0,
                        4.0 * ((double)rows_in * a->C * a->group_in * (a->x_up ? 1.5 : 1.0) + (double)rows * a->C * a->n_out));
    const size_t lds = ((size_t)a->n_out * (a->group_in * a->ksize + 3) + (a->pre_gamma ? 2 : 0)) * a->C * sizeof(float);
    static const int rw_env = [] { const char* e = getenv("VRD_DW_RW"); return e ? atoi(e) : 0; }();
    int rw = DW_RW;
    {
        const int64_t wgs_per_cu = lds ? (int64_t)(160 * 1024 / lds) : 8;
        const int64_t resident = 256 * (wgs_per_cu < 1 ? 1 : wgs_per_cu > 4 ? 4 : wgs_per_cu) * 4;
        auto strips_at = [&](int r) -> int64_t {
            return a->segs ? vrd::seg_table(sg, a->segs, a->stride, r) : (int64_t)a->B * ((Tout + r - 1) / r);
        };
        if (strips_at(DW_RW) < 6 * resident) {
            double best = 1e30;
            for (int r = 8; r <= 32; ++r) {
                const int64_t n = strips_at(r);
                const double cost = (double)((n + resident - 1) / resident) * (r + 3);
                if (cost < best - 1e-9) best = cost, rw = r;
            }
        }
        if (rw_env >= 1 && rw_env <= 64) rw = rw_env;
    }
    const int strips = (Tout + rw - 1) / rw;
    static const int spw_env = [] { const char* e = getenv("VRD_DW_SPW"); return e ? atoi(e) : 0; }();
    const int64_t total_strips = a->segs ? vrd::seg_table(sg, a->segs, a->stride, rw) : (int64_t)a->B * strips;
    const int spw = spw_env > 0 ? spw_env : 1;
    dim3 grid((unsigned)((total_strips + 4 * spw - 1) / (4 * spw))), block(256);
    bool any_f16 = false;
    for (int o = 0; o < a->n_out; ++o) any_f16 |= a->out_pair[o] == VRD_PAIR_F16;
    unsigned* const rflag = any_f16 ? vrd::range_flag() : nullptr;
#define VRD_DW(NV, KS, GIN) hipLaunchKernelGGL((dwconv_ln_kernel<NV, KS, GIN>), grid, block, lds, s, *a, Tout, strips, spw, rw, rflag, sg)
    if (a->group_in == 2) VRD_DW(1, 3, 2);
    else if (a->C == 256 && a->ksize == 3) VRD_DW(1, 3, 1);
    else if (a->C == 256) VRD_DW(1, 1, 1);
    else if (a->ksize == 3) VRD_DW(2, 3, 1);
    else VRD_DW(2, 1, 1);
#undef VRD_DW
    VRD_LAUNCH_CHECK();
    return 0;
}

int vrd_maxpool_mask(const float* x, int64_t ldx, int B, int Tin, int C, const uint8_t* mask_in, float* y, int64_t ldy,
                     uint8_t* mask_out, void* stream) {
    VRD_CHECK_ARG(x && y && mask_in, "vrd_maxpool_mask: null pointer");
    VRD_CHECK_ARG(B > 0 && Tin > 0 && Tin % 2 == 0 && C % 4 == 0, "vrd_maxpool_mask: Tin must be even, C %% 4 == 0");
    VRD_CHECK_ARG(ldx % 4 == 0 && ldy % 4 == 0 && ldx >= C && ldy >= C && aligned16(x) && aligned16(y), "vrd_maxpool_mask: bad layout");
    hipStream_t s = static_cast<hipStream_t>(stream);
    const int64_t n = (int64_t)B * (Tin / 2) * (C / 4);
    vrd::ProfScope prof(VRD_K_POOL, s, 0.0, 4.0 * (double)B * Tin * C * 1.5);
    hipLaunchKernelGGL(maxpool_mask_kernel, dim3((unsigned)((n + 255) / 256)), dim3(256), 0, s, x, ldx, B, Tin, C, mask_in, y, ldy, mask_out);
    VRD_LAUNCH_CHECK();
    return 0;
}

int vrd_mask_head(const float* emb, int64_t ld_emb, const float* feat, int64_t ld_feat, const uint8_t* out_mask, int B,
                  int Q, int T, int Dp, float fill, float* seg, void* stream) {
    VRD_CHECK_ARG(emb && feat && out_mask && seg, "vrd_mask_head: null pointer");
    VRD_CHECK_ARG(Dp == MH_D, "vrd_mask_head: mask dim must be %d (got %d)", MH_D, Dp);
    VRD_CHECK_ARG(Q >= 1 && Q <= MH_QMAX, "vrd_mask_head: num queries must be 1..%d (got %d)", MH_QMAX, Q);
    VRD_CHECK_ARG(B > 0 && B <= 65535 && T > 0, "vrd_mask_head: bad B/T");
    VRD_CHECK_ARG(ld_emb % 4 == 0 && ld_feat % 4 == 0 && aligned16(emb) && aligned16(feat), "vrd_mask_head: bad layout");
    hipStream_t s = static_cast<hipStream_t>(stream);
    vrd::ProfScope prof(VRD_K_MASK_HEAD, s, 2.0 * B * (double)Q * T * Dp, 4.0 * B * ((double)T * Dp + (double)Q * Dp + (double)Q * T));
    hipLaunchKernelGGL(mask_head_kernel, dim3((T + MH_TT - 1) / MH_TT, B), dim3(256), 0, s, emb, ld_emb, feat, ld_feat, out_mask, Q, T, fill, seg);
    VRD_LAUNCH_CHECK();
    return 0;
}

}
```

vrdone_amd/models/blocks.py:

```python
import math

import torch
from torch import nn

from .transformer import _get_activation_fn


def _ops():
    from .. import ops
    return ops


def _mask2d(mask):
    return mask.reshape(mask.shape[0], mask.shape[-1]).contiguous()


def _from_cl(x_cl):
    return _ops().btc_to_bct(x_cl)


def _to_cl(x):
    return _ops().to_channels_last(x)


# ... 78 lines not shown
                x = ops.conv_gemm(x, layer.weight, layer.bias, row_mask=row_mask, out=out, out_pair=out_pair, res=res)
        return x

    def forward(self, x):
        return _from_cl(self.cl(_to_cl(x)))


class _FactorPool:
    POOL = 4096

    def __init__(self):
        self.pools = {}

    def reset(self):
        self.pools.clear()

    def take(self, n, keep_prob, device):
        capturing = torch.cuda.is_current_stream_capturing()
        key = (device, keep_prob)
        ent = self.pools.get(key)
        if ent is None or ent[2] != capturing or ent[1] + n > ent[0].numel():
            size = max(self.POOL, n)
            ent = self.pools[key] = [torch.floor(keep_prob + torch.rand(size, device=device)) / keep_prob, 0, capturing]
        out = ent[0][ent[1]:ent[1] + n]
        ent[1] += n
        return out


_factor_pool = _FactorPool()


class AffineDropPath(nn.Module):

    def __init__(self, num_dim, drop_prob=0.0, init_scale_value=1e-4):
        super().__init__()
        self.scale = nn.Parameter(init_scale_value * torch.ones(1, num_dim, 1))
        self.drop_prob = drop_prob
        self.keep = None

    def row_factors(self, n_samples, rows_per_sample, device):
        if not self.training or self.drop_prob == 0.0 or not torch.is_grad_enabled():
            return None
        keep_prob = 1.0 - self.drop_prob
        if self.keep is not None:
            assert self.keep.numel() >= n_samples
            factors = self.keep[:n_samples].to(device=device, dtype=torch.float32) / keep_prob
        else:
            factors = _factor_pool.take(n_samples, keep_prob, torch.device(device))
        return factors[:, None].expand(n_samples, rows_per_sample).contiguous().view(-1)

    def forward(self, x):
        y = x * self.scale
        rf = self.row_factors(x.shape[0], 1, x.device)
        return y if rf is None else y * rf.view(-1, 1, 1)


class Scale(nn.Module):

    def __init__(self, init_value=1.0):
        super().__init__()
        self.scale = nn.Parameter(torch.tensor(init_value, dtype=torch.float32))

    def forward(self, x):
        return x * self.scale


class _ConvAttention(nn.Module):

    def _build(self, n_embd, n_head, q_kernel, kv_kernel, stride):
        assert n_embd % n_head == 0
        self.n_embd, self.n_head = n_embd, n_head
        self.n_channels = n_embd // n_head
        self.scale = 1.0 / math.sqrt(self.n_channels)
        for name, ks in (("query", q_kernel), ("key", kv_kernel), ("value", kv_kernel)):
            setattr(self, f"{name}_conv", MaskedConv1D(n_embd, n_embd, ks, stride=stride, padding=ks // 2,
                                                        groups=n_embd, bias=False))
            setattr(self, f"{name}_norm", LayerNorm(n_embd))
        self.key = nn.Conv1d(n_embd, n_embd, 1)
        self.query = nn.Conv1d(n_embd, n_embd, 1)
        self.value = nn.Conv1d(n_embd, n_embd, 1)
        self.attn_drop, self.proj_drop = nn.Dropout(0.0), nn.Dropout(0.0)
        self.proj = nn.Conv1d(n_embd, n_embd, 1)

    def _branch_set(self, name):
        conv, norm = getattr(self, f"{name}_conv"), getattr(self, f"{name}_norm")
        return dict(weight=conv.conv.weight, gamma=norm.weight, beta=norm.bias, pair=_ops().pair_mode())

    def _groups(self, q_in, k_in, v_in, q_mask, kv_mask, pre_ln=None, pre_ln_on="qkv"):
        specs = [("query", q_in, q_mask, "q"), ("key", k_in, kv_mask, "k"), ("value", v_in, kv_mask, "v")]
        groups = []
        for name, x, m, tag in specs:
            ks = getattr(self, f"{name}_conv").conv.kernel_size
            use_ln = pre_ln is not None and tag in pre_ln_on
            for g in groups:
                if g[0] is x and g[1] is m and g[2] == use_ln and g[3] == ks:
                    g[4].append(name)
                    break
            else:
                groups.append((x, m, use_ln, ks, [name]))
        return groups

    def _prep(self, q_in, k_in, v_in, q_mask, kv_mask, stride=1, pre_ln=None, pre_ln_on="qkv"):
        ops = _ops()
        outs = {}
        for x, m, use_ln, _, names in self._groups(q_in, k_in, v_in, q_mask, kv_mask, pre_ln, pre_ln_on):
            res = ops.dwconv_ln(x, [self._branch_set(n) for n in names], mask_out=m, stride=stride,
                                pre_ln=pre_ln if use_ln else None)
            outs.update(zip(names, res))
        return outs["query"], outs["key"], outs["value"]

    def _project(self, q, k, v, out_pair=False, q_mask=None, kv_mask=None):
        ops = _ops()
        return tuple(ops.conv_gemm_batch([
            ((q, self.query.weight, self.query.bias), dict(out_pair=out_pair, skip_rows=q_mask)),
            ((k, self.key.weight, self.key.bias), dict(out_pair=out_pair, skip_rows=kv_mask)),
            ((v, self.value.weight, self.value.bias), dict(out_pair=out_pair, skip_rows=kv_mask))]))


def make_rel_pe(n_embd, n_head, window_size):
    rel_pe = nn.Parameter(torch.zeros(1, 1, n_head, window_size))
    nn.init.trunc_normal_(rel_pe, std=(2.0 / n_embd) ** 0.5)
    return rel_pe


class LocalMaskedMHCA(_ConvAttention):

    def __init__(self, n_embd, n_head, window_size, n_qx_stride=1, n_kv_stride=1, attn_pdrop=0.0, proj_pdrop=0.0,
                 use_rel_pe=False):
        super().__init__()
        assert window_size > 1 and window_size % 2 == 1
        assert n_qx_stride == n_kv_stride and n_kv_stride in (1, 2)
        assert attn_pdrop == 0.0 and proj_pdrop == 0.0
        self.window_size, self.window_overlap = window_size, window_size // 2
        self.use_rel_pe = use_rel_pe
        self.n_qx_stride, self.n_kv_stride = n_qx_stride, n_kv_stride
        ks = n_kv_stride + 1 if n_kv_stride > 1 else 3
        self._build(n_embd, n_head, ks, ks, n_kv_stride)
        self.rel_pe = make_rel_pe(n_embd, n_head, window_size) if use_rel_pe else None

    def cl(self, x, mask, mask_out=None, pre_ln=None, **epilogue):
        ops = _ops()
        s = self.n_kv_stride
        if mask_out is None:
            mask_out = mask if s == 1 else mask[:, ::s].contiguous()
        q, k, v = self._prep(x, x, x, mask_out, mask_out, stride=s, pre_ln=pre_ln)
        q, k, v = self._project(q, k, v, q_mask=mask_out, kv_mask=mask_out)
        att = ops.local_attention(q, k, v, mask_out, self.n_head, self.window_overlap, pair=ops.pair_mode(),
                                  rel_pe=self.rel_pe)
        return ops.conv_gemm(att, self.proj.weight, self.proj.bias, row_mask=mask_out, **epilogue), mask_out

    def forward(self, x, mask):
        assert (x.shape[-1] // self.n_kv_stride) % (2 * self.window_overlap) == 0
        y, m = self.cl(_to_cl(x), _mask2d(mask))
        return _from_cl(y), m[:, None, :]


class MaskedMHCA(_ConvAttention):

    def __init__(self, n_embd, n_head, n_qx_stride=1, n_kv_stride=1, attn_pdrop=0.0, proj_pdrop=0.0):
        super().__init__()
        assert n_qx_stride == n_kv_stride and n_kv_stride in (1, 2), "built for equal query / key-value strides 1 or 2"
        assert attn_pdrop == 0.0 and proj_pdrop == 0.0
        self.n_qx_stride, self.n_kv_stride = n_qx_stride, n_kv_stride
        ks = n_kv_stride + 1 if n_kv_stride > 1 else 3
        self._build(n_embd, n_head, ks, ks, n_kv_stride)

    def cl(self, x, mask, mask_out=None, pre_ln=None, **epilogue):
        ops = _ops()
        s = self.n_kv_stride
        if mask_out is None:
            mask_out = mask if s == 1 else mask[:, ::s].contiguous()
        q, k, v = self._prep(x, x, x, mask_out, mask_out, stride=s, pre_ln=pre_ln)
        qkv_pair = ops.flash_pair_ok(self.n_head, self.n_embd, q.shape[1])
        q, k, v = self._project(q, k, v, out_pair=qkv_pair, q_mask=mask_out, kv_mask=mask_out)
        att = ops.attention(q, k, v, mask_out, self.n_head, pair=ops.pair_mode(), q_mask=mask_out)
        return ops.conv_gemm(att, self.proj.weight, self.proj.bias, row_mask=mask_out, **epilogue), mask_out

    def forward(self, x, mask):
        y, m = self.cl(_to_cl(x), _mask2d(mask))
        return _from_cl(y), m[:, None, :]


class MaskedMHA(nn.Module):

    def __init__(self, n_embd, n_head, attn_pdrop=0.0, proj_pdrop=0.0):
        super().__init__()
        assert n_embd % n_head == 0 and attn_pdrop == 0.0 and proj_pdrop == 0.0
        self.n_embd, self.n_head = n_embd, n_head
        self.n_channels = n_embd // n_head
        self.scale = 1.0 / math.sqrt(self.n_channels)
        self.key = nn.Conv1d(n_embd, n_embd, 1)
        self.query = nn.Conv1d(n_embd, n_embd, 1)
        self.value = nn.Conv1d(n_embd, n_embd, 1)
        self.attn_drop, self.proj_drop = nn.Dropout(0.0), nn.Dropout(0.0)
        self.proj = nn.Conv1d(n_embd, n_embd, 1)

    def cl_qkv(self, q_in, k_in, v_in, q_mask, kv_mask, **epilogue):
        ops = _ops()
        q = ops.conv_gemm(q_in, self.query.weight, self.query.bias)
        k = ops.conv_gemm(k_in, self.key.weight, self.key.bias)
        v = ops.conv_gemm(v_in, self.value.weight, self.value.bias)
        att = ops.attention(q, k, v, kv_mask, self.n_head)
        return ops.conv_gemm(att, self.proj.weight, self.proj.bias, row_mask=q_mask, **epilogue), q_mask

    def forward(self, x, mask):
        m = _mask2d(mask)
        xc = _to_cl(x)
        y, _ = self.cl_qkv(xc, xc, xc, m, m)
        return _from_cl(y), mask


class TransformerBlock(nn.Module):

    def __init__(self, n_embd, n_head, n_ds_strides=(1, 1), n_out=None, n_hidden=None, act_layer=nn.GELU,
                 attn_pdrop=0.0, proj_pdrop=0.0, path_pdrop=0.0, mha_win_size=-1, use_rel_pe=False):
        super().__init__()
        assert len(n_ds_strides) == 2 and act_layer is nn.GELU
        self.ln1 = LayerNorm(n_embd)
        self.ln2 = LayerNorm(n_embd)
        if mha_win_size > 1:
            self.attn = LocalMaskedMHCA(n_embd, n_head, window_size=mha_win_size, n_qx_stride=n_ds_strides[0],
                                        n_kv_stride=n_ds_strides[1], attn_pdrop=attn_pdrop, proj_pdrop=proj_pdrop,
                                        use_rel_pe=use_rel_pe)
        else:
            self.attn = MaskedMHCA(n_embd, n_head, n_qx_stride=n_ds_strides[0], n_kv_stride=n_ds_strides[1],
                                   attn_pdrop=attn_pdrop, proj_pdrop=proj_pdrop)
        s = n_ds_strides[0]
        self.pool_skip = nn.MaxPool1d(s + 1, stride=s, padding=(s + 1) // 2) if s > 1 else nn.Identity()
        n_hidden = n_hidden or 4 * n_embd
        n_out = n_out or n_embd
        assert n_out == n_embd
        self.mlp = nn.Sequential(nn.Conv1d(n_embd, n_hidden, 1), act_layer(), nn.Dropout(proj_pdrop, inplace=True),
                                 nn.Conv1d(n_hidden, n_out, 1), nn.Dropout(proj_pdrop, inplace=True))
        if path_pdrop > 0.0:
            self.drop_path_attn = AffineDropPath(n_embd, drop_prob=path_pdrop)
            self.drop_path_mlp = AffineDropPath(n_out, drop_prob=path_pdrop)
        else:
            self.drop_path_attn = nn.Identity()
            self.drop_path_mlp = nn.Identity()

    @staticmethod
    def _scale(dp):
        return dp.scale if isinstance(dp, AffineDropPath) else None

    @staticmethod
    def _drop(dp, mask):
        return dp.row_factors(mask.shape[0], mask.shape[1], mask.device) if isinstance(dp, AffineDropPath) else None

    def cl(self, x, mask, out=None):
        ops = _ops()
        if self.attn.n_kv_stride > 1:
            skip, m_out = ops.maxpool_mask(x, mask)
        else:
            skip, m_out = x, mask
        y, _ = self.attn.cl(x, mask, m_out, pre_ln=(self.ln1.weight, self.ln1.bias),
                            scale=self._scale(self.drop_path_attn), row_scale=self._drop(self.drop_path_attn, m_out),
                            res=skip, res_masked=True)
        h = self.ln2.cl(y, pair=ops.pair_mode())
        h = ops.conv_gemm(h, self.mlp[0].weight, self.mlp[0].bias, act=ops.ACT_GELU, out_pair=ops.pair_mode(), skip_rows=m_out)
        y = ops.conv_gemm(h, self.mlp[3].weight, self.mlp[3].bias, row_mask=m_out, scale=self._scale(self.drop_path_mlp),
                          row_scale=self._drop(self.drop_path_mlp, m_out), res=y, out=out)
        return y, m_out

    def forward(self, x, mask, pos_embd=None):
        assert pos_embd is None
        y, m = self.cl(_to_cl(x), _mask2d(mask))
        return _from_cl(y), m[:, None, :]
```

vrdone_amd/models/ragged.py:

```python
import torch

from .blocks import _ConvAttention, _ops


_MAX_SEGS = 32


class Layout:

    def __init__(self, buckets):
        self.segs, self.flat, off = [], [], 0
        self._tails = {}
        for n, T, flat in buckets:
            self.segs.append((off, n, T))
            self.flat.append(bool(flat))
            off += n * T
        assert self.flat == sorted(self.flat, reverse=True), "buckets that take the flat k = 3 convs come first"
        self.rows = off
        self.rows_flat = sum(n * T for (_, n, T), f in zip(self.segs, self.flat) if f)

    def twice(self):
        return self.segs + [(self.rows + off, n, T) for off, n, T in self.segs]

    def tail_rows(self, halves, device):
# ... 45 lines not shown
                      mask_out=_mpart(mask_out, oo, n, To), stride=stride, x_up=_part(x_up, off // 2, n, T // 2), pre_ln=pre_ln)
    else:
        for g0 in range(0, len(segs), _MAX_SEGS):
            part = segs[g0:g0 + _MAX_SEGS]
            r0, r1 = part[0][0], part[-1][0] + part[-1][1] * part[-1][2]
            rel = [(off - r0, n, T) for off, n, T in part]
            ops.dwconv_ln(x[:, r0:r1], [dict(st, out=b[:, r0 // stride:r1 // stride]) for st, b in zip(sets, bufs)],
                          mask_out=None if mask_out is None else mask_out[:, r0 // stride:r1 // stride], stride=stride,
                          x_up=None if x_up is None else x_up[:, r0 // 2:r1 // 2], pre_ln=pre_ln, segs=rel)
    return [ops.Pair(b, Cout) if ops._fmt(st.get("pair")) else b for st, b in zip(sets, bufs)]


def _attention_rows(q, k, v, kv_mask, q_mask, n_head, qsegs, ksegs, *, half_win=None, rel_pe=None, pair=False, plain=False):
    ops = _ops()
    Cc = q.shape[-1]
    out = torch.empty(1, sum(n * T for _, n, T in qsegs), Cc, device=_raw(q).device, dtype=torch.float32)
    r = None
    if len(qsegs) > 1 and len(_merged(qsegs)) == 1 and len(_merged(ksegs)) == 1:
        qsegs, ksegs = _merged(qsegs), _merged(ksegs)
    if half_win is not None and 1 < len(qsegs) <= _MAX_SEGS:
        assert list(qsegs) == list(ksegs)
        r = ops.local_attention(q, k, v, kv_mask, n_head, half_win, pair=pair, rel_pe=rel_pe, out=out, segs=list(qsegs))
        return ops.Pair(out, Cc, r.fmt) if isinstance(r, ops.Pair) else out
    dev = _raw(q).device
    lanes = _lanes(dev) if half_win is None and len(qsegs) > 2 else None
    if lanes:
        main = torch.cuda.current_stream(dev)
        ready = torch.cuda.Event()
        ready.record(main)
        for lane in lanes:
            lane.wait_event(ready)
    for i, ((qo, n, Tq), (ko, nk, Tk)) in enumerate(zip(qsegs, ksegs)):
        assert n == nk
        o = _part(out, qo, n, Tq)
        if lanes and i % (len(lanes) + 1):
            with torch.cuda.stream(lanes[i % (len(lanes) + 1) - 1]):
                r = _attention_one(q, k, v, kv_mask, q_mask, n_head, (qo, n, Tq), (ko, nk, Tk), o, pair, plain)
            continue
        if half_win is not None:
            assert Tq == Tk
            r = ops.local_attention(_part(q, qo, n, Tq), _part(k, ko, n, Tk), _part(v, ko, n, Tk), _mpart(kv_mask, ko, n, Tk),
                                    n_head, half_win, pair=pair, rel_pe=rel_pe, out=o)
        elif plain:
            r = ops.attention(_part(q, qo, n, Tq), _part(k, ko, n, Tk), _part(v, ko, n, Tk), _mpart(kv_mask, ko, n, Tk), n_head, out=o)
        else:
            r = ops.attention(_part(q, qo, n, Tq), _part(k, ko, n, Tk), _part(v, ko, n, Tk), _mpart(kv_mask, ko, n, Tk), n_head,
                              pair=pair, q_mask=_mpart(q_mask, qo, n, Tq), out=o)
    if lanes:
        for lane in lanes:
            main.wait_stream(lane)
    return ops.Pair(out, Cc, r.fmt) if isinstance(r, ops.Pair) else out


def _attention_one(q, k, v, kv_mask, q_mask, n_head, qseg, kseg, o, pair, plain):
    ops = _ops()
    (qo, n, Tq), (ko, _, Tk) = qseg, kseg
    if plain:
        return ops.attention(_part(q, qo, n, Tq), _part(k, ko, n, Tk), _part(v, ko, n, Tk), _mpart(kv_mask, ko, n, Tk), n_head, out=o)
    return ops.attention(_part(q, qo, n, Tq), _part(k, ko, n, Tk), _part(v, ko, n, Tk), _mpart(kv_mask, ko, n, Tk), n_head,
                         pair=pair, q_mask=_mpart(q_mask, qo, n, Tq), out=o)


ATTN_LANES = int(__import__("os").environ.get("VRDONE_ROWS_ATTN_STREAMS", "2"))
_side_streams = {}


def _lanes(dev):
    if ATTN_LANES <= 1 or torch.cuda.is_current_stream_capturing():
        return None
    key = (dev.index if dev.index is not None else torch.cuda.current_device(), ATTN_LANES)
    if key not in _side_streams:
        _side_streams[key] = [torch.cuda.Stream(device=dev) for _ in range(ATTN_LANES - 1)]
    return _side_streams[key]


def _attn_rows(mod, q_in, k_in, v_in, q_mask, kv_mask, qsegs, ksegs, *, stride=1, pre_ln=None, pre_ln_on="", **epilogue):
    ops = _ops()
    if stride > 1:
        qsegs_o = ksegs_o = [(off // stride, n, T // stride) for off, n, T in qsegs]
    else:
        qsegs_o, ksegs_o = qsegs, ksegs
    if isinstance(mod, _ConvAttention):
        outs = {}
        for x, m, use_ln, _, names in mod._groups(q_in, k_in, v_in, q_mask, kv_mask, pre_ln, pre_ln_on):
            res = _dwconv_rows(x, [mod._branch_set(nm) for nm in names], m, qsegs if x is q_in else ksegs, stride=stride,
                               pre_ln=pre_ln if use_ln else None)
            outs.update(zip(names, res))
        q, k, v = outs["query"], outs["key"], outs["value"]
        half_win = getattr(mod, "_half_win", None)
        if half_win is None and hasattr(mod, "window_overlap"):
            half_win = mod.window_overlap
        qkv_pair = half_win is None and ops.flash_pair_ok(mod.n_head, mod.n_embd, min(T for _, _, T in qsegs_o))
        q, k, v = mod._project(q, k, v, out_pair=qkv_pair, q_mask=q_mask, kv_mask=kv_mask)
        att = _attention_rows(q, k, v, kv_mask, q_mask, mod.n_head, qsegs_o, ksegs_o, half_win=half_win,
                              rel_pe=getattr(mod, "rel_pe", None), pair=ops.pair_mode())
    else:
        q = ops.conv_gemm(q_in, mod.query.weight, mod.query.bias)
        k = ops.conv_gemm(k_in, mod.key.weight, mod.key.bias)
        v = ops.conv_gemm(v_in, mod.value.weight, mod.value.bias)
        att = _attention_rows(q, k, v, kv_mask, None, mod.n_head, qsegs_o, ksegs_o, plain=True)
    return ops.conv_gemm(att, mod.proj.weight, mod.proj.bias, row_mask=q_mask, **epilogue)


def _block(blk, x, mask, segs, out=None):
    ops = _ops()
    s = blk.attn.n_kv_stride
    if s > 1:
        assert s == 2
        rows_o = sum(n * (T // 2) for _, n, T in segs)
        skip = torch.empty(1, rows_o, x.shape[-1], device=x.device, dtype=torch.float32)
        m_out = torch.empty(1, rows_o, device=x.device, dtype=torch.bool)
        for off, n, T in segs:
            ops.maxpool_mask(_part(x, off, n, T), _mpart(mask, off, n, T), out=(_part(skip, off // 2, n, T // 2), _mpart(m_out, off // 2, n, T // 2)))
        segs_o = [(off // 2, n, T // 2) for off, n, T in segs]
    else:
        skip, m_out, segs_o = x, mask, segs
    y = _attn_rows(blk.attn, x, x, x, m_out, m_out, segs, segs, stride=s, pre_ln=(blk.ln1.weight, blk.ln1.bias), pre_ln_on="qkv",
                   scale=blk._scale(blk.drop_path_attn), res=skip, res_masked=True)
    h = blk.ln2.cl(y, pair=ops.pair_mode())
    h = ops.conv_gemm(h, blk.mlp[0].weight, blk.mlp[0].bias, act=ops.ACT_GELU, out_pair=ops.pair_mode(), skip_rows=m_out)
    y = ops.conv_gemm(h, blk.mlp[3].weight, blk.mlp[3].bias, row_mask=m_out, scale=blk._scale(blk.drop_path_mlp), res=y, out=out)
    return y, m_out, segs_o


def _decoder_layer(layer, tgt, memory, tgt_mask, memory_mask, qsegs, ksegs, *, query_pos=None, stream_add=None, out=None):
    ops = _ops()
    from .local_transformer import MaskedMHCA_QKV
    fuse1 = query_pos is None and isinstance(layer.self_attn, MaskedMHCA_QKV)
    fuse2 = query_pos is None and isinstance(layer.multihead_attn, MaskedMHCA_QKV)
    last = not layer.with_ffn
    kw1 = dict(scale=layer._scale(layer.drop_path_attn1), res=tgt, res_masked=True)
    if fuse1:
        tgt = _attn_rows(layer.self_attn, tgt, tgt, tgt, tgt_mask, tgt_mask, qsegs, qsegs, pre_ln=(layer.ln1.weight, layer.ln1.bias),
                         pre_ln_on="qk", **kw1)
    else:
        t2 = layer.ln1.cl(tgt, post_add=query_pos)
        tgt = _attn_rows(layer.self_attn, t2, t2, tgt, tgt_mask, tgt_mask, qsegs, qsegs, **kw1)
    kw = dict(scale=layer._scale(layer.drop_path_attn2), res=tgt, res_masked=True, res2=stream_add if last else None,
              out=out if last else None)
    if fuse2:
        tgt = _attn_rows(layer.multihead_attn, tgt, memory, memory, tgt_mask, memory_mask, qsegs, ksegs,
                         pre_ln=(layer.ln2.weight, layer.ln2.bias), pre_ln_on="q", **kw)
    else:
        t2 = layer.ln2.cl(tgt, post_add=query_pos)
        tgt = _attn_rows(layer.multihead_attn, t2, memory, memory, tgt_mask, memory_mask, qsegs, ksegs, **kw)
    if layer.with_ffn:
        assert stream_add is None
        t2 = layer.ln3.cl(tgt)
        h = ops.conv_gemm(t2, layer.mlp[0].weight, layer.mlp[0].bias, act=ops.ACT_GELU)
        tgt = ops.conv_gemm(h, layer.mlp[3].weight, layer.mlp[3].bias, row_mask=tgt_mask, scale=layer._scale(layer.drop_path_mlp),
                            res=tgt, out=out)
    return tgt


def _rows_of(x, sl):
    ops = _ops()
    return ops.Pair(x.t[:, sl], x.width, x.fmt) if isinstance(x, ops.Pair) else x[:, sl]


def _conv3_rows(h, conv, row_mask, lay, halves, tails, out=None, out_pair=False, norm=None):
    ops = _ops()
    assert conv.kernel_size[0] == 3
    N = conv.weight.shape[0]
    if out is None:
        out = torch.empty(1, halves * lay.rows, N, device=_raw(h).device, dtype=torch.float32)
    if tails is not None:
        _zero_rows(h, tails)
    small = ops.conv_ln_ok(h, conv.weight, conv.bias, *((norm.weight, norm.bias) if norm is not None else ()))
    assert small or norm is None

    def one(x, m, o):
        if small:
            ops.conv_ln(x, conv.weight, conv.bias, row_mask=m, out=o, pair=out_pair, relu=norm is not None,
                        gamma=None if norm is None else norm.weight.reshape(-1), beta=None if norm is None else norm.bias.reshape(-1))
        else:
            ops.conv_gemm(x, conv.weight, conv.bias, row_mask=m, out=o, out_pair=out_pair)
    for hf in range(halves):
        base = hf * lay.rows
        if lay.rows_flat:
            sl = slice(base, base + lay.rows_flat)
            one(_rows_of(h, sl), row_mask[:, sl], out[:, sl])
        for (off, n, T), flat in zip(lay.segs, lay.flat):
            if not flat:
                one(_part(h, base + off, n, T), _mpart(row_mask, base + off, n, T), _part(out, base + off, n, T))
    return ops.Pair(out, N) if out_pair else out


def _embed(h, convs, norms, mask2, out, lay, tails2):
    ops = _ops()
    last = len(convs) - 1
    if last == 0 and ops.conv_ln_ok(h, convs[0].conv.weight, convs[0].conv.bias, norms[0].weight, norms[0].bias):
        return _conv3_rows(h, convs[0].conv, mask2, lay, 2, tails2, out=out, out_pair=bool(ops.pair_mode()), norm=norms[0])
    for i, (conv, norm) in enumerate(zip(convs, norms)):
        h = _conv3_rows(h, conv.conv, mask2, lay, 2, tails2)
        h = norm.cl(h, relu=True, out=out if i == last else None, pair=ops.pair_mode())
    return h


def unpack_rows(bb, x, plan, lay):
    ops = _ops()
    R = lay.rows
    V, Cc, S, E = bb.n_visual, bb.n_clip, bb.n_bbox_so, bb.n_bbox_entity
    pair = ops.pair_mode()
    new = lambda rows, width: torch.empty(1, rows, width, device=x.device, dtype=torch.float32)
# ... 185 lines not shown
```

vrdone_amd/ops.py:

```python
import ctypes as C
import os

import torch

from . import _hip
from ._hip import ACT_GELU, ACT_NONE, ACT_RELU, lib


_raw_stream = getattr(torch._C, "_cuda_getCurrentRawStream", None)


def _stream():
    if _raw_stream is not None:
        return C.c_void_p(_raw_stream(torch.cuda.current_device()))
    return C.c_void_p(torch.cuda.current_stream().cuda_stream)


def _rows(t):
    if not t.is_cuda:
        raise RuntimeError("vrdone_amd ops need HIP tensors (no CPU path exists for the hot path)")
    if t.dtype != torch.float32:
        raise TypeError(f"expected float32, got {t.dtype}")
    if t.stride(-1) != 1:
        raise ValueError("channels-last operand must have unit stride along channels")
# ... 483 lines not shown
    vis, so_box, ent, mask = bufs[:4]
    clip = bufs[4] if Cc else None
    assert vis.shape == (2 * B, T, V) and so_box.shape == (B, T, S) and ent.shape == (2 * B, T, E) and mask.shape == (B, T)
    assert mask.dtype == torch.bool and all(t.is_contiguous() and t.device == dev for t in bufs)
    for t in (source.vis, source.clip, source.boxes):
        assert t is None or (t.is_contiguous() and t.dtype == torch.float32 and t.device == dev)
    targets = torch.empty(G, T, device=dev, dtype=torch.float32)
    a = _hip.GatherTrainArgs()
    a.vis, a.clip, a.boxes = source.vis.data_ptr(), _ptr(source.clip), source.boxes.data_ptr()
    a.s_row, a.o_row, a.lens, a.lead = d["s_row"].data_ptr(), d["o_row"].data_ptr(), d["lens"].data_ptr(), d["lead"].data_ptr()
    a.seq_wh, a.seg_lo, a.seg_hi = d["seq_wh"].data_ptr(), d["seg_lo"].data_ptr(), d["seg_hi"].data_ptr()
    a.P, a.G, a.T, a.V, a.Cc, a.stride = B, G, T, V, Cc, tables.stride
    a.out_vis, a.out_clip, a.out_so_box, a.out_ent = vis.data_ptr(), _ptr(clip), so_box.data_ptr(), ent.data_ptr()
    a.out_mask, a.out_targets = mask.data_ptr(), targets.data_ptr()
    a.pair_wide = _fmt(pair_wide)
    _hip.check(lib.vrd_gather_train(C.byref(a), _stream()), "vrd_gather_train")
    if a.pair_wide:
        vis = Pair(vis, V, a.pair_wide)
        clip = Pair(clip, Cc, a.pair_wide) if Cc else None
    return vis, clip, so_box, ent, mask, targets


def assemble_pairs(streams, snippets, stream_row, lens, T, piece, reach):
    P = lens.shape[0]
    D = streams.shape[-1]
    L = snippets.shape[1]
    assert snippets.shape == (4 * P, L, D) and stream_row.shape == (2 * P,) and stream_row.dtype == torch.int64
    assert lens.dtype == torch.int32 and streams.is_contiguous() and snippets.is_contiguous()
    out = torch.empty(2 * P, T, D, device=streams.device, dtype=torch.float32)
    a = _hip.AssembleArgs()
    a.streams, a.snippets, a.stream_row, a.lens = streams.data_ptr(), snippets.data_ptr(), stream_row.data_ptr(), lens.data_ptr()
    a.P, a.T, a.D, a.L, a.piece, a.reach = P, T, D, L, piece, reach
    a.out = out.data_ptr()
    _hip.check(lib.vrd_assemble_pairs(C.byref(a), _stream()), "vrd_assemble_pairs")
    return out


def btc_to_bct(x):
    if recording(x):
        from . import autograd
        return autograd.FromChannelsLast.apply(x)
    B, T, Cc = x.shape
    p, rows, cols, ld = _rows(x)
    out = torch.empty(B, Cc, T, device=x.device, dtype=torch.float32)
    _hip.check(lib.vrd_btc_to_bct(p, ld, B, Cc, T, out.data_ptr(), _stream()), "vrd_btc_to_bct")
    return out


def to_channels_last(x):
    if recording(x):
        from . import autograd
        return autograd.ToChannelsLast.apply(x)
    B, Cc, T = x.shape
    out = torch.empty(B, T, Cc, device=x.device, dtype=torch.float32)
    return bct_to_btc(x.contiguous(), 0, Cc, out)


_skip_padding = os.environ.get("VRDONE_SKIP_PADDING", "1") != "0"
SKIP_MIN_ROWS = 65536


def row_blocks(mask):
    hit = getattr(mask, "_vrd_row_blocks", None)
    key = (mask.data_ptr(), mask._version)
    capturing = _capturing()
    if hit is not None and hit[0] == key and not capturing:
        return hit[1]
    rows = mask.numel()
    val = None
    if rows % 32 == 0 and mask.is_contiguous() and mask.data_ptr() % 16 == 0 and mask.dtype in (torch.bool, torch.uint8):
        nblk = rows // 32
        seg_len = 8 * (((nblk + 7) // 8 + 7) // 8)
        order = torch.empty(nblk, device=mask.device, dtype=torch.int32)
        count = torch.empty((nblk + seg_len - 1) // seg_len, device=mask.device, dtype=torch.int32)
        _hip.check(lib.vrd_row_blocks(mask.data_ptr(), rows, seg_len, order.data_ptr(), count.data_ptr(), _stream()),
                   "vrd_row_blocks")
        val = (order, count, seg_len)
    if capturing:
        return _keep_for_capture(val)
    mask._vrd_row_blocks = (key, val)
    return val


def conv_gemm(x, weight, bias=None, *, act=ACT_NONE, row_mask=None, scale=None, res=None, res_masked=False,
              res2=None, out=None, out_pair=False, skip_rows=None, row_scale=None, _launch=None, _dgrad=False, _split_fmt=None,
              _a_scale=None, _bfmt=None, _family=None):
    if _launch is None and not isinstance(x, Pair) and (recording(x, weight, bias, scale, res, res2) or row_scale is not None):
        from . import autograd
        assert not out_pair
        return autograd.conv_gemm(x, weight, bias, act=act, row_mask=row_mask, scale=scale, row_scale=row_scale, res=res,
                                  res_masked=res_masked, res2=res2)
    assert row_scale is None, "row_scale (drop-path sampling) exists for plain f32 rows only"
    N, Cin, k = weight.shape
    if _dgrad:
        N, Cin = Cin, N
    x_fmt = x.fmt if isinstance(x, Pair) else 0
    x, a_width = _unwrap(x)
    pa, rows, cols, lda = _rows(x)
    assert cols == Cin, f"input has {cols} channels, weight expects {Cin}"
    T = x.shape[-2]
    if out is None:
        out = torch.empty(*x.shape[:-1], N, device=x.device, dtype=torch.float32)
    pc, rows_c, cols_c, ldc = _rows(out)
    assert rows_c == rows and cols_c == N
    a = _hip.GemmArgs()
    if _dgrad:
        assert (Cin * k) % 32 == 0 and not a_width
        wt = split_conv_weight_dgrad(weight, _bfmt)
        a.W = wt.data_ptr()
        wt.set_args(a)
        if wt.fmt == _hip.PAIR_F16:
            assert _a_scale is not None
            a.a_scale = _a_scale.data_ptr()
    else:
        a.W = _param_ptr(packed_conv_weight(weight), x, "conv weight")
    a.A, a.lda, a.bias = pa, lda, _param_ptr(bias, x, "conv bias")
    a.C, a.ldc = pc, ldc
    a.M, a.N, a.Cin, a.taps, a.T = rows, N, Cin, k, T
    a.act = act
    a.row_mask = _mask_ptr(row_mask, rows)
    a.scale = _param_ptr(scale, x, "drop-path scale")
    if a_width:
        assert pair_fmt() and x_fmt == pair_fmt() and Cin % 32 == 0, "pair input needs the split-precision mode it was made in and Cin % 32 == 0"
    w_fmt = pair_fmt() if _split_fmt is None else _split_fmt
    if _dgrad:
        w_fmt = a.split_fmt
    assert not (a_width and w_fmt != x_fmt) and not (out_pair and w_fmt != pair_fmt())
    if not _dgrad and w_fmt and (Cin * k) % 32 == 0:
        split_conv_weight(weight, w_fmt).set_args(a)
        if w_fmt == _hip.PAIR_F16 and _split_fmt is None:
            a.products = products()
    a.a_pair_width = a_width
    a.c_pair = _fmt(out_pair)
    if skip_rows is None:
        skip_rows = row_mask
    f32_kernel = not a_width and not _dgrad and not (w_fmt and (Cin * k) % 32 == 0)
    if _skip_padding and skip_rows is not None and (a_width or f32_kernel) and rows >= SKIP_MIN_ROWS and skip_rows.numel() == rows:
        blocks = row_blocks(skip_rows)
        if blocks is not None:
            a.row_blocks, a.row_blocks_active = blocks[0].data_ptr(), blocks[1].data_ptr()
            a.row_block_seg_len = blocks[2]
    if res is not None:
        pr, rr, rc, ldr = _rows(res)
        assert rr == rows and rc == N
        a.res, a.ldres, a.res_masked = pr, ldr, 1 if res_masked else 0
    if res2 is not None:
        pr, rr, rc, ldr = _rows(res2)
        assert rr == rows and rc == N
        a.res2, a.ldres2 = pr, ldr
    if _family is not None:
        fam = lib.vrd_gemm_family(C.byref(a))
        if fam < 0:
            _hip.check(fam, "vrd_gemm_family")
        _family.append(fam)
    if _launch is not None:
        _launch.append(a)
    else:
        _hip.check(lib.vrd_gemm(C.byref(a), _stream()), "vrd_gemm")
    return Pair(out, N, a.c_pair) if a.c_pair else out


def split_forward(x, weight, bias=None, **kwargs):
    family = []
    conv_gemm(x, weight, bias, _launch=[], _family=family, **kwargs)
    return family[0] != _hip.K_GEMM


def conv_gemm_batch(calls):
    assert 1 <= len(calls) <= 4
    if torch.is_grad_enabled():
        return [conv_gemm(*args, **kwargs) for args, kwargs in calls]
    collected, results = [], []
    for args, kwargs in calls:
        results.append(conv_gemm(*args, _launch=collected, **kwargs))
    arr = (_hip.GemmArgs * len(collected))(*collected)
    _hip.check(lib.vrd_gemm_batch(arr, len(collected), _stream()), "vrd_gemm_batch")
    return results


def layernorm(x, gamma, beta, *, relu=False, post_add=None, out=None, pair=False):
    if recording(x, gamma, beta, post_add):
        from . import autograd
        assert not pair
        return autograd.layernorm(x, gamma, beta, relu=relu, post_add=post_add)
    px, rows, cols, ldx = _rows(x)
    if out is None:
        out = torch.empty(*x.shape, device=x.device, dtype=torch.float32)
    py, rows_y, cols_y, ldy = _rows(out)
    assert rows_y == rows and cols_y == cols
    pa, lda, period = None, 0, 0
    if post_add is not None:
        pa, period, ca, lda = _rows(post_add)
        assert ca == cols
    assert gamma.numel() == cols and beta.numel() == cols
    _hip.check(lib.vrd_layernorm(px, ldx, py, ldy, rows, cols, _param_ptr(gamma, x, "LayerNorm weight"),
                                 _param_ptr(beta, x, "LayerNorm bias"), 1 if relu else 0,
                                 pa, lda, period, _fmt(pair), _stream()), "vrd_layernorm")
    return Pair(out, cols) if _fmt(pair) else out


CONV_LN_MAXK = 32
_conv_ln_on = os.environ.get("VRDONE_CONV_LN", "1") != "0"


def conv_ln_ok(x, weight, *tensors):
    N, Cin, k = weight.shape
    return (_conv_ln_on and not isinstance(x, Pair) and k in (1, 3) and Cin * k <= CONV_LN_MAXK and (3 + k) * Cin <= 64 and N in (256, 512) and
            not recording(x, weight, *tensors))


def conv_ln(x, weight, bias, *, row_mask=None, gamma=None, beta=None, relu=False, out=None, pair=False):
    N, Cin, k = weight.shape
    px, rows, cols, ldx = _rows(x)
    assert cols == Cin and weight.is_contiguous()
    if out is None:
        out = torch.empty(*x.shape[:-1], N, device=x.device, dtype=torch.float32)
    py, rows_y, cols_y, ldy = _rows(out)
    assert rows_y == rows and cols_y == N
    a = _hip.ConvLnArgs()
    a.x, a.ldx, a.rows = px, ldx, rows
    a.Cin, a.taps, a.T, a.N = Cin, k, x.shape[-2], N
    a.w, a.bias = _param_ptr(weight, x, "conv weight"), _param_ptr(bias, x, "conv bias")
    a.row_mask = _mask_ptr(row_mask, rows)
    a.gamma, a.beta = _param_ptr(gamma, x, "LayerNorm weight"), _param_ptr(beta, x, "LayerNorm bias")
    a.relu = 1 if relu else 0
    a.y, a.ldy, a.out_pair = py, ldy, _fmt(pair)
    _hip.check(lib.vrd_conv_ln(C.byref(a), _stream()), "vrd_conv_ln")
    return Pair(out, N) if a.out_pair else out


_CONST_ROWS = {}


def _const_row(n, fill, device):
    key = (n, float(fill), str(device))
    t = _CONST_ROWS.get(key)
    if t is None:
        t = _CONST_ROWS[key] = torch.full((n,), fill, device=device, dtype=torch.float32)
    return t


def _dwconv_block(w, bias, gamma, beta):
    parts = (w, bias, gamma, beta)
    key = tuple((t.data_ptr(), t._version) if t is not None else None for t in parts)
    hit = getattr(w, "_vrd_dw_block", None)
    capturing = _capturing()
    if hit is not None and hit[0] == key and not capturing:
        return hit[1]
    Cout, g, k = w.shape
    one = lambda t, fill: _const_row(Cout, fill, w.device) if t is None else t.detach().float().reshape(-1)
    val = torch.cat([w.detach().float().permute(1, 2, 0).reshape(-1), one(bias, 0.0), one(gamma, 1.0), one(beta, 0.0)]).contiguous()
    if capturing:
        return _keep_for_capture(val)
    w._vrd_dw_block = (key, val)
    return val


def dwconv_ln(x, sets, *, mask_out=None, stride=1, x_up=None, pre_ln=None, segs=None):
    if recording(x, x_up, *(t for st in sets for t in (st["weight"], st.get("bias"), st.get("gamma"), st.get("beta"))),
                 *(pre_ln or ())):
        from . import autograd
        return autograd.dwconv_ln(x, sets, mask_out=mask_out, stride=stride, x_up=x_up, pre_ln=pre_ln)
    B, Tin, Cx = x.shape
    w0 = sets[0]["weight"]
    Cout, g, k = w0.shape
    px, rows, cols, ldx = _rows(x)
    assert cols == Cout * g
    Tout = Tin // stride
    a = _hip.DwconvLnArgs()
    seg_table = None
    if segs is not None:
        assert B == 1 and sum(n * T for _, n, T in segs) == Tin
        seg_table = _hip.RowSegs.of(segs)
        a.segs = C.pointer(seg_table)
    a.x, a.ldx = px, ldx
    if x_up is not None:
        pu, ru, cu, ldu = _rows(x_up)
        assert cu == cols and ru * 2 == rows
        a.x_up, a.ldx_up = pu, ldu
    a.B, a.Tin, a.C, a.ksize, a.stride, a.group_in = B, Tin, Cout, k, stride, g
    if pre_ln is not None:
        assert g == 1 and x_up is None
        a.pre_gamma, a.pre_beta = _param_ptr(pre_ln[0], x, "LayerNorm weight"), _param_ptr(pre_ln[1], x, "LayerNorm bias")
    a.mask_out = _mask_ptr(mask_out, B * Tout)
    a.n_out = len(sets)
    outs, blocks = [], []
    for i, s in enumerate(sets):
        assert tuple(s["weight"].shape) == (Cout, g, k) and s["weight"].is_contiguous()
        o = s.get("out")
        if o is None:
            o = torch.empty(B, Tout, Cout, device=x.device, dtype=torch.float32)
        po, ro, co, ldo = _rows(o)
        assert ro == B * Tout and co == Cout
        a.w[i], a.bias[i] = _param_ptr(s["weight"], x, "depthwise weight"), _param_ptr(s.get("bias"), x, "depthwise bias")
        a.gamma[i], a.beta[i] = (_param_ptr(s.get("gamma"), x, "LayerNorm weight"),
                                 _param_ptr(s.get("beta"), x, "LayerNorm bias"))
        blocks.append(_dwconv_block(s["weight"], s.get("bias"), s.get("gamma"), s.get("beta")))
        a.packed[i] = blocks[-1].data_ptr()
        a.relu[i] = 1 if s.get("relu") else 0
        a.y[i], a.ldy[i] = po, ldo
        a.out_pair[i] = _fmt(s.get("pair"))
        outs.append(Pair(o, Cout) if _fmt(s.get("pair")) else o)
    _hip.check(lib.vrd_dwconv_ln(C.byref(a), _stream()), "vrd_dwconv_ln")
    return outs


def _rel_pe_ptr(rel_pe, like, n_head, half_win):
    if rel_pe is None:
        return None
    assert rel_pe.numel() == n_head * (2 * half_win + 1) and rel_pe.dtype == torch.float32 and rel_pe.is_contiguous()
    assert rel_pe.device == like.device
    return rel_pe.data_ptr()


def local_attention(q, k, v, mask, n_head, half_win, pair=False, rel_pe=None, out=None, segs=None):
    if recording(q, k, v, rel_pe):
        from . import autograd
        return autograd.LocalAttention.apply(q, k, v, mask, n_head, half_win, rel_pe)
    B, T, Cc = q.shape
    rel = _rel_pe_ptr(rel_pe, q, n_head, half_win)
    pq, rows, cols, ld = _rows(q)
    pk, _, _, ldk = _rows(k)
    pv, _, _, ldv = _rows(v)
    assert ld == ldk == ldv
    if out is None:
        out = torch.empty(B, T, Cc, device=q.device, dtype=torch.float32)
    assert out.shape == (B, T, Cc) and out.is_contiguous()
    if segs is not None:
        assert B == 1 and sum(n * t for _, n, t in segs) == T
        table = _hip.RowSegs.of(segs)
        _hip.check(lib.vrd_local_attn_segs(pq, pk, pv, ld, _mask_ptr(mask, rows), rel, C.byref(table), Cc, n_head, half_win,
                                           out.data_ptr(), Cc, _fmt(pair), _stream()), "vrd_local_attn_segs")
        return Pair(out, Cc) if _fmt(pair) else out
    _hip.check(lib.vrd_local_attn(pq, pk, pv, ld, _mask_ptr(mask, rows), rel, B, T, Cc, n_head, half_win,
                                  out.data_ptr(), Cc, _fmt(pair), _stream()), "vrd_local_attn")
    return Pair(out, Cc) if _fmt(pair) else out


def attention(q, k, v, kv_mask, n_head, algo=0, pair=False, q_mask=None, out=None):
    if not isinstance(q, Pair) and recording(q, k, v):
        from . import autograd
        return autograd.Attention.apply(q, k, v, kv_mask, n_head)
    if isinstance(q, Pair):
        assert isinstance(k, Pair) and isinstance(v, Pair) and q.width == k.width == v.width == q.shape[-1]
        assert q.fmt == k.fmt == v.fmt
        fmt = q.fmt
        q, k, v = q.t, k.t, v.t
        B, Tq, Cc = q.shape
        Tk = k.shape[1]
        pq, _, _, ldq = _rows(q)
        pk, rows_k, _, ldk = _rows(k)
        pv, _, _, ldv = _rows(v)
        assert ldk == ldv
        if out is None:
            out = torch.empty(B, Tq, Cc, device=q.device, dtype=torch.float32)
        assert out.shape == (B, Tq, Cc) and out.is_contiguous()
        _hip.check(lib.vrd_attention_pair(pq, ldq, pk, pv, ldk, _mask_ptr(kv_mask, rows_k), _mask_ptr(q_mask, B * Tq), B, Tq, Tk, n_head,
                                          Cc // n_head, out.data_ptr(), Cc, fmt if pair else 0, fmt, _stream(),
                                          products() if fmt == _hip.PAIR_F16 else 0),
                   "vrd_attention_pair")
        return Pair(out, Cc, fmt) if pair else out
    B, Tq, Cc = q.shape
    Tk = k.shape[1]
    pq, _, _, ldq = _rows(q)
    pk, rows_k, _, ldk = _rows(k)
    pv, _, _, ldv = _rows(v)
    assert ldk == ldv
    if out is None:
        out = torch.empty(B, Tq, Cc, device=q.device, dtype=torch.float32)
    assert out.shape == (B, Tq, Cc) and out.is_contiguous()
    hd = Cc // n_head
    flash = algo == 2 or (algo == 0 and hd in (64, 128))
    pair = bool(pair and flash and pair_fmt())
    _hip.check(lib.vrd_attention(pq, ldq, pk, pv, ldk, _mask_ptr(kv_mask, rows_k), B, Tq, Tk, n_head, hd,
                                 out.data_ptr(), Cc, algo, _fmt(pair), _stream()), "vrd_attention")
    return Pair(out, Cc) if pair else out


def maxpool_mask(x, mask_in, out=None):
    if recording(x):
        from . import autograd
        return autograd.MaxPoolMask.apply(x, mask_in)
    B, T, Cc = x.shape
    px, rows, cols, ldx = _rows(x)
# ... 84 lines not shown
```

Before: 15640.

## Skip writing and reading fully padded row blocks in inference GEMMs and dwconv

Adds a dead-rows contract. Producers (the MLP up-projection GEMM and the dwconv+LN q/k/v outputs) no longer write 32-row blocks that are entirely padding, and consumers (the QKV projection and the MLP down-projection in the big x3 kernel) stop loading those rows by using a zero-size buffer resource. Producer and consumer must agree, so the downstream GEMM has to mask them. This saves memory traffic and epilogue work on padded frames, but leaves those buffers holding uninitialised data, so it is limited to inference with no grad and to shapes the 256x256 kernel handles.

After: 15730 (median of 6 runs). No clear change (+0.6%).

```diff
diff --git a/include/vrdone_hip.h b/include/vrdone_hip.h
--- a/include/vrdone_hip.h
+++ b/include/vrdone_hip.h
@@ -121,11 +121,13 @@
     const int32_t* row_blocks;
     const int32_t* row_blocks_active;
     int32_t row_block_seg_len;
+    int32_t dead_rows;
     int32_t split_fmt;
     const float* w_scale;
     const float* a_scale;
     int32_t products;
 } vrd_gemm_args;
+enum vrd_dead_rows { VRD_DEAD_C = 1, VRD_DEAD_A = 2 };
 int vrd_gemm(const vrd_gemm_args* a, void* stream);
 int vrd_gemm_family(const vrd_gemm_args* a);
 int vrd_gemm_batch(const vrd_gemm_args* a, int count, void* stream);
@@ -179,6 +181,7 @@
     const float* pre_beta;
     const float* packed[3];
     const vrd_row_segs* segs;
+    int32_t y_dead[3];
 } vrd_dwconv_ln_args;
 int vrd_dwconv_ln(const vrd_dwconv_ln_args* a, void* stream);
 
diff --git a/vrdone_amd/_hip.py b/vrdone_amd/_hip.py
--- a/vrdone_amd/_hip.py
+++ b/vrdone_amd/_hip.py
@@ -41,10 +41,11 @@
                 ("res", c_f32p), ("ldres", C.c_int64), ("res_masked", C.c_int32),
                 ("res2", c_f32p), ("ldres2", C.c_int64), ("W_split", C.c_void_p),
                 ("a_pair_width", C.c_int32), ("c_pair", C.c_int32),
-                ("row_blocks", C.c_void_p), ("row_blocks_active", C.c_void_p), ("row_block_seg_len", C.c_int32),
+                ("row_blocks", C.c_void_p), ("row_blocks_active", C.c_void_p), ("row_block_seg_len", C.c_int32), ("dead_rows", C.c_int32),
                 ("split_fmt", C.c_int32), ("w_scale", c_f32p), ("a_scale", c_f32p), ("products", C.c_int32)]
 
 
+DEAD_C, DEAD_A = 1, 2
 MAX_SEGS = 32
 
 
@@ -75,7 +76,8 @@
                 ("mask_out", c_u8p), ("n_out", C.c_int32),
                 ("w", c_f32p * 3), ("bias", c_f32p * 3), ("gamma", c_f32p * 3), ("beta", c_f32p * 3),
                 ("relu", C.c_int32 * 3), ("y", c_f32p * 3), ("ldy", C.c_int64 * 3), ("out_pair", C.c_int32 * 3),
-                ("pre_gamma", c_f32p), ("pre_beta", c_f32p), ("packed", c_f32p * 3), ("segs", C.POINTER(RowSegs))]
+                ("pre_gamma", c_f32p), ("pre_beta", c_f32p), ("packed", c_f32p * 3), ("segs", C.POINTER(RowSegs)),
+                ("y_dead", C.c_int32 * 3)]
 
 
 class ConvLnArgs(C.Structure):
diff --git a/vrdone_amd/csrc/vrd_gemm.hip b/vrdone_amd/csrc/vrd_gemm.hip
--- a/vrdone_amd/csrc/vrd_gemm.hip
+++ b/vrdone_amd/csrc/vrd_gemm.hip
@@ -260,6 +260,8 @@
                                      a->row_block_seg_len % 8 == 0),
                   "vrd_gemm: a row-block list needs its active counts, M %% 32 == 0 and a segment length that is a multiple of 8 (M = %lld, seg_len %d)",
                   (long long)a->M, a->row_block_seg_len);
+    VRD_CHECK_ARG((a->dead_rows & ~(VRD_DEAD_C | VRD_DEAD_A)) == 0 && (!a->dead_rows || a->row_blocks),
+                  "vrd_gemm: dead_rows (%d) takes VRD_DEAD_C | VRD_DEAD_A and needs a row-block list", a->dead_rows);
     return 0;
 }
 }
@@ -295,6 +297,8 @@
                                 (1.0 + (a->res ? 1.0 : 0.0) + (a->res2 ? 1.0 : 0.0)));
     const X3Choice pick = choose_x3(a, vec, staged);
     const bool x3 = pick.x3, dma = pick.dma, big = pick.big;
+    VRD_CHECK_ARG(!(a->dead_rows & VRD_DEAD_A) || big, "vrd_gemm: VRD_DEAD_A needs a GEMM the 256 x 256 split-precision kernel takes (M=%lld N=%d K=%d)",
+                  (long long)a->M, a->N, K);
     vrd::ProfScope prof(big ? VRD_K_GEMM_X3_BIG : dma ? VRD_K_GEMM_X3_DMA : (x3 ? VRD_K_GEMM_X3 : VRD_K_GEMM), s, flops, bytes);
     if (x3) {
         int rc3 = big ? vrd::launch_gemm_x3_big(*a, s)
@@ -331,7 +335,7 @@
                x.act == y.act && x.row_mask == y.row_mask && x.scale == y.scale && x.res == y.res && x.ldres == y.ldres &&
                x.res_masked == y.res_masked && x.res2 == y.res2 && x.ldres2 == y.ldres2 && x.a_pair_width == y.a_pair_width &&
                x.c_pair == y.c_pair && x.row_blocks == y.row_blocks && x.row_blocks_active == y.row_blocks_active &&
-               x.row_block_seg_len == y.row_block_seg_len && (x.bias != nullptr) == (y.bias != nullptr) &&
+               x.row_block_seg_len == y.row_block_seg_len && x.dead_rows == y.dead_rows && (x.bias != nullptr) == (y.bias != nullptr) &&
                (x.W_split != nullptr) == (y.W_split != nullptr) && x.split_fmt == y.split_fmt;
     }
     static const int batch_env = [] { const char* e = getenv("VRD_GEMM_BATCH"); return e ? atoi(e) : 1; }();
diff --git a/vrdone_amd/csrc/vrd_gemm_epilogue.h b/vrdone_amd/csrc/vrd_gemm_epilogue.h
--- a/vrdone_amd/csrc/vrd_gemm_epilogue.h
+++ b/vrdone_amd/csrc/vrd_gemm_epilogue.h
@@ -91,7 +91,8 @@
 
 template <bool ROWIN, int ACT, int SLAB, int ROWS, typename Transposer>
 __device__ __forceinline__ void gemm_epilogue_lean_tr(const vrd_gemm_args& p, Transposer&& transpose_into, float* stg, int64_t mw,
-                                                      int64_t mw1, int nw, int lane, const EpiCols& cols, unsigned* rflag = nullptr) {
+                                                      int64_t mw1, int nw, int lane, const EpiCols& cols, unsigned* rflag = nullptr,
+                                                      bool first_only = false) {
     RangeTrack rt;
     const int64_t hop = mw1 - (mw + 32);
     const int c4 = (lane & 15) * 4, rb0 = lane >> 4;
@@ -139,6 +140,7 @@
     transpose_into(stg, SLAB == 64 ? -1 : 0);
 #pragma unroll
     for (int pass = 0; pass < NPASS; ++pass) {
+        if (pass == 2 && first_only) break;
         if (SLAB == 32 && pass == 2) transpose_into(stg, 1);
         const RowIn cur = q0;
         q0 = q1;
@@ -230,7 +232,8 @@
 
 template <bool ROWIN, int ACT, int SLAB = 64>
 __device__ __forceinline__ void gemm_epilogue_lean16(const vrd_gemm_args& p, const f32x4_t (&acc)[4][4], float* stg, int64_t mw,
-                                                     int64_t mw1, int nw, int lane, const EpiCols& cols, unsigned* rflag = nullptr) {
+                                                     int64_t mw1, int nw, int lane, const EpiCols& cols, unsigned* rflag = nullptr,
+                                                     bool first_only = false) {
     const int lc = lane & 15, lq = lane >> 4;
     gemm_epilogue_lean_tr<ROWIN, ACT, SLAB, 64>(
         p,
@@ -245,7 +248,7 @@
                     for (int j = 0; j < 4; ++j) slab[(r0 + 4 * lq + j) * STG_PITCH + (tj ^ lq) * 16 + lc] = acc[ti][tj][j];
             }
         },
-        stg, mw, mw1, nw, lane, cols, rflag);
+        stg, mw, mw1, nw, lane, cols, rflag, first_only);
 }
 
 inline bool gemm_epilogue_lean_ok(const vrd_gemm_args& a) {
diff --git a/vrdone_amd/csrc/vrd_gemm_x3_big.hip b/vrdone_amd/csrc/vrd_gemm_x3_big.hip
--- a/vrdone_amd/csrc/vrd_gemm_x3_big.hip
+++ b/vrdone_amd/csrc/vrd_gemm_x3_big.hip
@@ -121,7 +121,7 @@
     const int wm = WH, wn = wave & 3;
     auto blk_of = [&](int slot) { return slot < nblk ? (rb ? vrd::uniform_load(rb + slot) : slot) : -1; };
     struct Tile {
-        int tm, n0;
+        int tm, n0, nact;
         bool contract;
     };
     auto tile_of = [&](int vb_) {
@@ -131,10 +131,12 @@
         t.tm = lid / tiles_n;
         t.n0 = (lid - t.tm * tiles_n) * TN;
         t.contract = true;
+        t.nact = 8;
         if (rb) {
             const int seg_len = p.row_block_seg_len;
             const int seg = (t.tm * 8) / seg_len;
-            t.contract = t.tm * 8 < nblk && t.tm * 8 - seg * seg_len < vrd::uniform_load(p.row_blocks_active + seg);
+            t.nact = t.tm * 8 < nblk ? vrd::uniform_load(p.row_blocks_active + seg) - (t.tm * 8 - seg * seg_len) : 0;
+            t.contract = t.nact > 0;
         }
         return t;
     };
@@ -160,7 +162,8 @@
         __amdgpu_buffer_rsrc_t ra, rw;
     };
     auto src_of = [&](const Tile& t) {
-        const int my_blk = blk_of(t.tm * 8 + wave);
+        const bool a_dead = (p.dead_rows & VRD_DEAD_A) && wave >= t.nact;
+        const int my_blk = a_dead ? -1 : blk_of(t.tm * 8 + wave);
         const int64_t a_row = (int64_t)(my_blk < 0 ? 0 : my_blk) * 32 + rin;
         Src r;
         r.tseq0 = (TAPS == 3) ? (int)(a_row % p.T) : 0;
@@ -168,7 +171,7 @@
         const int w_in = (p.N - t.n0 - wave * PER * 8 + 7) / 8;
         r.w_last = (w_in > 0 ? (w_in < PER ? w_in : PER) : 1) - 1;
         const int64_t a_row_u = (int64_t)(my_blk < 0 ? 0 : my_blk) * 32 - (TAPS == 3 ? 1 : 0);
-        r.ra = __builtin_amdgcn_make_buffer_rsrc(const_cast<float*>(p.A + a_row_u * p.lda), 0, 0x80000000u, 0x00020000);
+        r.ra = __builtin_amdgcn_make_buffer_rsrc(const_cast<float*>(p.A + a_row_u * p.lda), 0, a_dead ? 0u : 0x80000000u, 0x00020000);
         r.rw = __builtin_amdgcn_make_buffer_rsrc(
             const_cast<char*>(reinterpret_cast<const char*>(p.W_split) + (int64_t)(t.n0 + (w_in > 0 ? wave * PER * 8 : 0)) * K * 4), 0,
             0x80000000u, 0x00020000);
@@ -214,7 +217,7 @@
 #else
     constexpr bool CARRY = true;
 #endif
-    Tile nt_keep = Tile{0, 0, false};
+    Tile nt_keep = Tile{0, 0, 0, false};
     Src nx_keep = src_of(nt_keep);
     do {
     if (PERSIST) {
@@ -227,6 +230,15 @@
     const Tile tile = (PERSIST && staged && CARRY) ? nt_keep : tile_of(vb);
     const int tm = tile.tm, n0 = tile.n0;
     const bool contract = tile.contract;
+    const bool dead_c = (p.dead_rows & VRD_DEAD_C) != 0;
+    const int nact = dead_c ? tile.nact : 8;
+    if (!contract && tid == 0 && tm * 8 < nblk)
+        atomicAdd(&g_big_skipped_kn, (unsigned long long)K * (unsigned)(p.N - n0 < TN ? p.N - n0 : TN));
+    if (!contract && dead_c) {
+        if (!PERSIST) return;
+        vq += (int)gridDim.x;
+        continue;
+    }
     const Src cur = (PERSIST && staged && CARRY) ? nx_keep : src_of(tile);
     bool next_staged = false;
     Src nx = cur;
@@ -239,8 +251,6 @@
         }
     }
     nx_keep = nx;
-    if (!contract && tid == 0 && tm * 8 < nblk)
-        atomicAdd(&g_big_skipped_kn, (unsigned long long)K * (unsigned)(p.N - n0 < TN ? p.N - n0 : TN));
 
     const int l15 = lane & 15, l4 = lane >> 4;
     int a_hi_off = (wm * 128 + l15) * ROWB + ((l4 ^ swz(l15)) * 16), a_lo_off = a_hi_off ^ 64;
@@ -401,7 +411,8 @@
         const int slot = tm * 8 + wm * 4 + hm * 2;
         const int blk_a = blk_of(slot), blk_b = blk_of(slot + 1);
         const int nw = n0 + wn * 64;
-        if (blk_a < 0 || nw >= p.N) {
+        const int live = nact - (wm * 4 + hm * 2);
+        if (blk_a < 0 || nw >= p.N || live <= 0) {
             all_stored = false;
             continue;
         }
@@ -412,9 +423,11 @@
         for (int i = 0; i < 4; ++i)
 #pragma unroll
             for (int j = 0; j < 4; ++j) part[i][j] = acc[4 * hm + i][j];
-        if (rowin) vrd::gemm_epilogue_lean16<true, VRD_ACT_NONE, SLAB>(p, part, stg, mw, mw1, nw, lane_e, cols, rflag);
-        else if (p.act == VRD_ACT_GELU) vrd::gemm_epilogue_lean16<false, VRD_ACT_GELU, SLAB>(p, part, stg, mw, mw1, nw, lane_e, cols, rflag);
-        else vrd::gemm_epilogue_lean16<false, VRD_ACT_NONE, SLAB>(p, part, stg, mw, mw1, nw, lane_e, cols, rflag);
+        const bool first_only = live == 1;
+        if (first_only) all_stored = false;
+        if (rowin) vrd::gemm_epilogue_lean16<true, VRD_ACT_NONE, SLAB>(p, part, stg, mw, mw1, nw, lane_e, cols, rflag, first_only);
+        else if (p.act == VRD_ACT_GELU) vrd::gemm_epilogue_lean16<false, VRD_ACT_GELU, SLAB>(p, part, stg, mw, mw1, nw, lane_e, cols, rflag, first_only);
+        else vrd::gemm_epilogue_lean16<false, VRD_ACT_NONE, SLAB>(p, part, stg, mw, mw1, nw, lane_e, cols, rflag, first_only);
     }
     LAB_STAMP(3);
     LAB_REAL(5);
diff --git a/vrdone_amd/csrc/vrd_rowops.hip b/vrdone_amd/csrc/vrd_rowops.hip
--- a/vrdone_amd/csrc/vrd_rowops.hip
+++ b/vrdone_amd/csrc/vrd_rowops.hip
@@ -335,7 +335,7 @@
 
 template <int NV, int KS, int GIN>
 __global__ __launch_bounds__(256) void dwconv_ln_kernel(vrd_dwconv_ln_args p, int Tout_u, int strips_per_seq, int strips_per_wave, int rw, unsigned* rflag,
-                                                        vrd::SegTable sg) {
+                                                        vrd::SegTable sg, int64_t out_rows) {
     vrd::RangeTrack rt;
     constexpr int C = 256 * NV, NT = GIN * KS, SETF = (NT + 3) * C;
     constexpr bool WIDE = NV == 2 && GIN == 1;
@@ -415,9 +415,16 @@
         const int64_t r0 = orow0 + to0;
         const bool mine = lane < to1 - to0 && p.mask_out[r0 + lane] != 0;
         if (!__any(mine)) {
+            bool dead_blk = false;
+            if (p.y_dead[0] | p.y_dead[1] | p.y_dead[2]) {
+                const int64_t b0 = r0 & ~(int64_t)31, b1 = min(((r0 + (to1 - to0) - 1) | 31) + 1, out_rows);
+                const bool live = b0 + lane < b1 && p.mask_out[b0 + lane] != 0;
+                dead_blk = b1 - b0 <= 64 && !__any(live);
+            }
 #pragma unroll
             for (int o = 0; o < 3; ++o) {
                 if (o >= p.n_out) break;
+                if (dead_blk && p.y_dead[o]) continue;
                 const float* const lb = dw_lds + o * SETF + (NT + 2) * C;
                 float4 val[NV];
 #pragma unroll
@@ -794,6 +801,7 @@
                           a->ldy[o] % 4 == 0 && a->ldy[o] >= a->C,
                       "vrd_dwconv_ln: bad output set %d", o);
         VRD_CHECK_ARG((a->gamma[o] == nullptr) == (a->beta[o] == nullptr), "vrd_dwconv_ln: gamma/beta mismatch");
+        VRD_CHECK_ARG(!a->y_dead[o] || a->mask_out, "vrd_dwconv_ln: y_dead needs mask_out");
     }
     vrd::SegTable sg;
     sg.count = 0;
@@ -841,7 +849,7 @@
     bool any_f16 = false;
     for (int o = 0; o < a->n_out; ++o) any_f16 |= a->out_pair[o] == VRD_PAIR_F16;
     unsigned* const rflag = any_f16 ? vrd::range_flag() : nullptr;
-#define VRD_DW(NV, KS, GIN) hipLaunchKernelGGL((dwconv_ln_kernel<NV, KS, GIN>), grid, block, lds, s, *a, Tout, strips, spw, rw, rflag, sg)
+#define VRD_DW(NV, KS, GIN) hipLaunchKernelGGL((dwconv_ln_kernel<NV, KS, GIN>), grid, block, lds, s, *a, Tout, strips, spw, rw, rflag, sg, rows)
     if (a->group_in == 2) VRD_DW(1, 3, 2);
     else if (a->C == 256 && a->ksize == 3) VRD_DW(1, 3, 1);
     else if (a->C == 256) VRD_DW(1, 1, 1);
diff --git a/vrdone_amd/models/blocks.py b/vrdone_amd/models/blocks.py
--- a/vrdone_amd/models/blocks.py
+++ b/vrdone_amd/models/blocks.py
@@ -184,9 +184,12 @@
         self.attn_drop, self.proj_drop = nn.Dropout(0.0), nn.Dropout(0.0)
         self.proj = nn.Conv1d(n_embd, n_embd, 1)
 
-    def _branch_set(self, name):
+    def _branch_set(self, name, dead=False):
         conv, norm = getattr(self, f"{name}_conv"), getattr(self, f"{name}_norm")
-        return dict(weight=conv.conv.weight, gamma=norm.weight, beta=norm.bias, pair=_ops().pair_mode())
+        return dict(weight=conv.conv.weight, gamma=norm.weight, beta=norm.bias, pair=_ops().pair_mode(), dead=dead)
+
+    def _dead(self, q_in, k_in, v_in, q_mask, kv_mask):
+        return q_mask is kv_mask and _ops().dead_rows_ok(q_mask, self.n_embd, self.training)
 
     def _groups(self, q_in, k_in, v_in, q_mask, kv_mask, pre_ln=None, pre_ln_on="qkv"):
         specs = [("query", q_in, q_mask, "q"), ("key", k_in, kv_mask, "k"), ("value", v_in, kv_mask, "v")]
@@ -202,21 +205,21 @@
                 groups.append((x, m, use_ln, ks, [name]))
         return groups
 
-    def _prep(self, q_in, k_in, v_in, q_mask, kv_mask, stride=1, pre_ln=None, pre_ln_on="qkv"):
+    def _prep(self, q_in, k_in, v_in, q_mask, kv_mask, stride=1, pre_ln=None, pre_ln_on="qkv", dead=False):
         ops = _ops()
         outs = {}
         for x, m, use_ln, _, names in self._groups(q_in, k_in, v_in, q_mask, kv_mask, pre_ln, pre_ln_on):
-            res = ops.dwconv_ln(x, [self._branch_set(n) for n in names], mask_out=m, stride=stride,
+            res = ops.dwconv_ln(x, [self._branch_set(n, dead) for n in names], mask_out=m, stride=stride,
                                 pre_ln=pre_ln if use_ln else None)
             outs.update(zip(names, res))
         return outs["query"], outs["key"], outs["value"]
 
-    def _project(self, q, k, v, out_pair=False, q_mask=None, kv_mask=None):
+    def _project(self, q, k, v, out_pair=False, q_mask=None, kv_mask=None, dead_in=False):
         ops = _ops()
         return tuple(ops.conv_gemm_batch([
-            ((q, self.query.weight, self.query.bias), dict(out_pair=out_pair, skip_rows=q_mask)),
-            ((k, self.key.weight, self.key.bias), dict(out_pair=out_pair, skip_rows=kv_mask)),
-            ((v, self.value.weight, self.value.bias), dict(out_pair=out_pair, skip_rows=kv_mask))]))
+            ((q, self.query.weight, self.query.bias), dict(out_pair=out_pair, skip_rows=q_mask, dead_in=dead_in)),
+            ((k, self.key.weight, self.key.bias), dict(out_pair=out_pair, skip_rows=kv_mask, dead_in=dead_in)),
+            ((v, self.value.weight, self.value.bias), dict(out_pair=out_pair, skip_rows=kv_mask, dead_in=dead_in))]))
 
 
 def make_rel_pe(n_embd, n_head, window_size):
@@ -245,8 +248,9 @@
         s = self.n_kv_stride
         if mask_out is None:
             mask_out = mask if s == 1 else mask[:, ::s].contiguous()
-        q, k, v = self._prep(x, x, x, mask_out, mask_out, stride=s, pre_ln=pre_ln)
-        q, k, v = self._project(q, k, v, q_mask=mask_out, kv_mask=mask_out)
+        dead = self._dead(x, x, x, mask_out, mask_out)
+        q, k, v = self._prep(x, x, x, mask_out, mask_out, stride=s, pre_ln=pre_ln, dead=dead)
+        q, k, v = self._project(q, k, v, q_mask=mask_out, kv_mask=mask_out, dead_in=dead)
         att = ops.local_attention(q, k, v, mask_out, self.n_head, self.window_overlap, pair=ops.pair_mode(),
                                   rel_pe=self.rel_pe)
         return ops.conv_gemm(att, self.proj.weight, self.proj.bias, row_mask=mask_out, **epilogue), mask_out
@@ -272,9 +276,10 @@
         s = self.n_kv_stride
         if mask_out is None:
             mask_out = mask if s == 1 else mask[:, ::s].contiguous()
-        q, k, v = self._prep(x, x, x, mask_out, mask_out, stride=s, pre_ln=pre_ln)
+        dead = self._dead(x, x, x, mask_out, mask_out)
+        q, k, v = self._prep(x, x, x, mask_out, mask_out, stride=s, pre_ln=pre_ln, dead=dead)
         qkv_pair = ops.flash_pair_ok(self.n_head, self.n_embd, q.shape[1])
-        q, k, v = self._project(q, k, v, out_pair=qkv_pair, q_mask=mask_out, kv_mask=mask_out)
+        q, k, v = self._project(q, k, v, out_pair=qkv_pair, q_mask=mask_out, kv_mask=mask_out, dead_in=dead)
         att = ops.attention(q, k, v, mask_out, self.n_head, pair=ops.pair_mode(), q_mask=mask_out)
         return ops.conv_gemm(att, self.proj.weight, self.proj.bias, row_mask=mask_out, **epilogue), mask_out
 
@@ -359,9 +364,11 @@
                             scale=self._scale(self.drop_path_attn), row_scale=self._drop(self.drop_path_attn, m_out),
                             res=skip, res_masked=True)
         h = self.ln2.cl(y, pair=ops.pair_mode())
-        h = ops.conv_gemm(h, self.mlp[0].weight, self.mlp[0].bias, act=ops.ACT_GELU, out_pair=ops.pair_mode(), skip_rows=m_out)
+        dead = ops.dead_rows_ok(m_out, y.shape[-1], self.training)
+        h = ops.conv_gemm(h, self.mlp[0].weight, self.mlp[0].bias, act=ops.ACT_GELU, out_pair=ops.pair_mode(), skip_rows=m_out,
+                          dead_out=dead)
         y = ops.conv_gemm(h, self.mlp[3].weight, self.mlp[3].bias, row_mask=m_out, scale=self._scale(self.drop_path_mlp),
-                          row_scale=self._drop(self.drop_path_mlp, m_out), res=y, out=out)
+                          row_scale=self._drop(self.drop_path_mlp, m_out), res=y, out=out, dead_in=dead)
         return y, m_out
 
     def forward(self, x, mask, pos_embd=None):
diff --git a/vrdone_amd/models/ragged.py b/vrdone_amd/models/ragged.py
--- a/vrdone_amd/models/ragged.py
+++ b/vrdone_amd/models/ragged.py
@@ -151,8 +151,9 @@
         qsegs_o, ksegs_o = qsegs, ksegs
     if isinstance(mod, _ConvAttention):
         outs = {}
+        dead = mod._dead(q_in, k_in, v_in, q_mask, kv_mask) and all(off % 32 == 0 for off, _, _ in qsegs_o)
         for x, m, use_ln, _, names in mod._groups(q_in, k_in, v_in, q_mask, kv_mask, pre_ln, pre_ln_on):
-            res = _dwconv_rows(x, [mod._branch_set(nm) for nm in names], m, qsegs if x is q_in else ksegs, stride=stride,
+            res = _dwconv_rows(x, [mod._branch_set(nm, dead) for nm in names], m, qsegs if x is q_in else ksegs, stride=stride,
                                pre_ln=pre_ln if use_ln else None)
             outs.update(zip(names, res))
         q, k, v = outs["query"], outs["key"], outs["value"]
@@ -160,7 +161,7 @@
         if half_win is None and hasattr(mod, "window_overlap"):
             half_win = mod.window_overlap
         qkv_pair = half_win is None and ops.flash_pair_ok(mod.n_head, mod.n_embd, min(T for _, _, T in qsegs_o))
-        q, k, v = mod._project(q, k, v, out_pair=qkv_pair, q_mask=q_mask, kv_mask=kv_mask)
+        q, k, v = mod._project(q, k, v, out_pair=qkv_pair, q_mask=q_mask, kv_mask=kv_mask, dead_in=dead)
         att = _attention_rows(q, k, v, kv_mask, q_mask, mod.n_head, qsegs_o, ksegs_o, half_win=half_win,
                               rel_pe=getattr(mod, "rel_pe", None), pair=ops.pair_mode())
     else:
@@ -187,8 +188,10 @@
     y = _attn_rows(blk.attn, x, x, x, m_out, m_out, segs, segs, stride=s, pre_ln=(blk.ln1.weight, blk.ln1.bias), pre_ln_on="qkv",
                    scale=blk._scale(blk.drop_path_attn), res=skip, res_masked=True)
     h = blk.ln2.cl(y, pair=ops.pair_mode())
-    h = ops.conv_gemm(h, blk.mlp[0].weight, blk.mlp[0].bias, act=ops.ACT_GELU, out_pair=ops.pair_mode(), skip_rows=m_out)
-    y = ops.conv_gemm(h, blk.mlp[3].weight, blk.mlp[3].bias, row_mask=m_out, scale=blk._scale(blk.drop_path_mlp), res=y, out=out)
+    dead = ops.dead_rows_ok(m_out, y.shape[-1], blk.training)
+    h = ops.conv_gemm(h, blk.mlp[0].weight, blk.mlp[0].bias, act=ops.ACT_GELU, out_pair=ops.pair_mode(), skip_rows=m_out, dead_out=dead)
+    y = ops.conv_gemm(h, blk.mlp[3].weight, blk.mlp[3].bias, row_mask=m_out, scale=blk._scale(blk.drop_path_mlp), res=y, out=out,
+                      dead_in=dead)
     return y, m_out, segs_o
 
 
diff --git a/vrdone_amd/ops.py b/vrdone_amd/ops.py
--- a/vrdone_amd/ops.py
+++ b/vrdone_amd/ops.py
@@ -589,15 +589,32 @@
     return val
 
 
+_dead_rows = os.environ.get("VRDONE_DEAD_ROWS", "1") != "0"
+_BIG_MIN_TILES = int(os.environ.get("VRD_X3_BIG_MIN_TILES", "512"))
+dead_rows_set = 0
+
+
+def dead_rows_ok(mask, channels, training=False):
+    if not (_dead_rows and _skip_padding and pair_fmt()) or mask is None or training or torch.is_grad_enabled():
+        return False
+    rows = mask.numel()
+    if rows < SKIP_MIN_ROWS or rows % 64 or channels % 64 or channels < 256 or mask.device.type != "cuda":
+        return False
+    if ((rows + 255) // 256) * ((channels + 255) // 256) < _BIG_MIN_TILES:
+        return False
+    return row_blocks(mask) is not None
+
+
 def conv_gemm(x, weight, bias=None, *, act=ACT_NONE, row_mask=None, scale=None, res=None, res_masked=False,
-              res2=None, out=None, out_pair=False, skip_rows=None, row_scale=None, _launch=None, _dgrad=False, _split_fmt=None,
-              _a_scale=None, _bfmt=None, _family=None):
+              res2=None, out=None, out_pair=False, skip_rows=None, row_scale=None, dead_out=False, dead_in=False, _launch=None,
+              _dgrad=False, _split_fmt=None, _a_scale=None, _bfmt=None, _family=None):
     if _launch is None and not isinstance(x, Pair) and (recording(x, weight, bias, scale, res, res2) or row_scale is not None):
         from . import autograd
         assert not out_pair
         return autograd.conv_gemm(x, weight, bias, act=act, row_mask=row_mask, scale=scale, row_scale=row_scale, res=res,
                                   res_masked=res_masked, res2=res2)
     assert row_scale is None, "row_scale (drop-path sampling) exists for plain f32 rows only"
+    assert not ((dead_out or dead_in) and torch.is_grad_enabled()), "dead rows are an inference-only contract"
     N, Cin, k = weight.shape
     if _dgrad:
         N, Cin = Cin, N
@@ -647,6 +664,13 @@
         if blocks is not None:
             a.row_blocks, a.row_blocks_active = blocks[0].data_ptr(), blocks[1].data_ptr()
             a.row_block_seg_len = blocks[2]
+            if _dead_rows:
+                a.dead_rows = (_hip.DEAD_C if dead_out else 0) | (_hip.DEAD_A if dead_in else 0)
+    if dead_in and not a.dead_rows & _hip.DEAD_A:
+        raise RuntimeError("conv_gemm: dead_in without a padding map -- the input's padded rows were never written")
+    if a.dead_rows:
+        global dead_rows_set
+        dead_rows_set += 1
     if res is not None:
         pr, rr, rc, ldr = _rows(res)
         assert rr == rows and rc == N
@@ -807,6 +831,11 @@
         a.relu[i] = 1 if s.get("relu") else 0
         a.y[i], a.ldy[i] = po, ldo
         a.out_pair[i] = _fmt(s.get("pair"))
+        if s.get("dead") and _dead_rows:
+            assert mask_out is not None and not torch.is_grad_enabled()
+            a.y_dead[i] = 1
+            global dead_rows_set
+            dead_rows_set += 1
         outs.append(Pair(o, Cout) if _fmt(s.get("pair")) else o)
     _hip.check(lib.vrd_dwconv_ln(C.byref(a), _stream()), "vrd_dwconv_ln")
     return outs
```
